# timmeinhardt/trackformer

Hardware: AMD Instinct MI355X
Metric: frames/sec, TrackFormer-Deformable inference (ResNet-50, 1333x800, 300 object + 100 track queries, bs 1 per GPU); roofline = ms_deform_attn HBM GB/s (higher is better)
Workload: dtype f32 (dense layers as the fp16 split product on MFMA: two fp16 pieces per activation, three per weight scaled per output channel -- 22 + 1 significand bits per operand, the one dropped product < 2^-22 --, three terms, f32 accumulate)

## Files before the change

include/tf_fused.h:

```cpp
#ifndef TF_FUSED_H_
#define TF_FUSED_H_

#include <stdint.h>

#ifdef __cplusplus
extern "C" {
#endif

int tf_bias_act_f32(float *x, const float *bias, const float *residual, int64_t n, int C, int relu,
                    void *stream);

int tf_add_layernorm_f32(const float *x, const float *res, const float *gamma, const float *beta,
                         float *out, int64_t rows, int C, float eps, void *stream);

int tf_box_refine_f32(const float *delta, const float *ref, float *out, int64_t rows, int ref_dim, float eps, void *stream);

int tf_postprocess_pack_f32(const float *logits, const float *boxes, float *out, int64_t Q, int C, float img_h, float img_w,
                            int clip, void *stream);

int tf_groupnorm_nhwc_f32(const float *x, const float *gamma, const float *beta, float *out, double *workspace, int N,
                          int HW, int C, int G, float eps, int64_t x_image_stride, int64_t out_image_stride, void *stream);
int tf_groupnorm_stats_nhwc_f32(const float *x, double *workspace, int N, int HW, int C, int G, int64_t x_image_stride, void *stream);
int tf_groupnorm_relu_nhwc_f32(const float *x, const float *gamma, const float *beta, float *out, double *workspace, int N,
                               int HW, int C, int G, float eps, int64_t x_image_stride, int64_t out_image_stride, void *stream);

int tf_upsample_add_nhwc_f32(const float *low, const float *fpn, float *out, int N, int q_per_image, int h, int w, int H, int W, int C,
                             void *stream);

int tf_conv3x3_merge_packed_f32(const float *low, const float *fpn, const double *gn_workspace, const float *gamma, const float *beta,
                                int groups, float eps, const void *w_packed, const float *bias, float *y, int nimg, int q_per_image, int lh,
                                int lw, int H, int W, int cin, int cout, int relu, int terms, void *stream);

int tf_groupnorm_relu_conv3x3_c1_nhwc_f32(const float *x, const float *gamma, const float *beta, const float *weight, float bias,
                                          float *out, double *workspace, int N, int H, int W, int C, int G, float eps, void *stream);

int tf_mask_label_map_f32(const float *logits, const int *order, int16_t *label, int n_tracks, int h, int w, int pad_h, int pad_w, int img_h,
                          int img_w, int out_h, int out_w, float threshold, void *stream);


int tf_linear_split_f32(const float *x, const void *w_hi, const void *w_mid, const void *w_lo, const float *w_scale, const float *bias,
                        float *y, int64_t M, int K, int N, int relu, void *stream);

int tf_linear_split_res_f32(const float *x, const void *w_hi, const void *w_mid, const void *w_lo, const float *w_scale, const float *bias,
                            const float *residual, float *y, int64_t M, int K, int N, int relu, void *stream);

int tf_conv3x3_split_f32(const float *x, const void *w_hi, const void *w_mid, const void *w_lo, const float *w_scale, const float *bias,
                         float *y, int nimg, int hin, int win, int cin, int cout, int stride, int relu, void *stream);
int tf_conv3x3_splitk_f32(const float *x, const void *w_hi, const void *w_mid, const void *w_lo, const float *w_scale, const float *bias,
                          float *y, float *workspace, int ksplit, int nimg, int hin, int win, int cin, int cout, int stride, int relu,
                          void *stream);
int tf_conv1x1_strided_split_f32(const float *x, const void *w_hi, const void *w_mid, const void *w_lo, const float *w_scale,
                                 const float *bias, float *y, int nimg, int hin, int win, int cin, int cout, int stride, int relu,
                                 void *stream);
int tf_conv1x1_splitk_f32(const float *x, const void *w_hi, const void *w_mid, const void *w_lo, const float *w_scale, const float *bias,
                          float *y, float *workspace, int ksplit, int nimg, int hin, int win, int cin, int cout, int stride, int relu,
                          void *stream);

int tf_stem_conv7x7_f32(const float *x, const void *w_packed, const float *bias, float *y, int N, int H, int W, int relu,
                        int terms, void *stream);

int tf_bias_relu_maxpool_f32(const float *x, const float *bias, float *out, int N, int H, int W, int C, void *stream);

int tf_linear_split_add_f32(const float *x, const float *x2, const void *w_hi, const void *w_mid, const void *w_lo, const float *w_scale,
                            const float *bias, float *y, int64_t M, int K, int N, void *stream);

int64_t tf_linear_packed_bytes(int K, int N, int terms);
int tf_linear_pack_weight_f32(const float *w, void *packed, int K, int N, int terms, void *stream);
int tf_linear_packed_f32(const float *x, const void *w_packed, const float *bias, const float *residual, float *y, int64_t M, int K,
                         int N, int relu, int terms, void *stream);

int tf_conv_packed_f32(const float *x, const void *w_packed, const float *bias, const float *residual, float *y, float *workspace,
                       int ksplit, int nimg, int hin, int win, int cin, int cout, int ks, int stride, int relu, int terms,
                       void *stream);

int tf_linear_res_ln_f32(const float *x, const void *w_packed, const float *bias, const float *residual, const float *ln_weight,
                         const float *ln_bias, float ln_eps, float *y, int64_t M, int K, int N, int terms, void *stream);

int tf_ffn_fused_f32(const float *x, const void *w1_packed, const float *b1, const void *w2_packed, const float *b2,
                     const float *residual, const float *ln_weight, const float *ln_bias, float ln_eps, float *y, int64_t M,
                     int d_model, int d_ffn, int terms, void *stream);

int tf_mha_core_f32(const float *q, const float *k, const float *v, float *out, const unsigned char *key_mask,
                    int N, int Lq, int Lk, int H, int D, int ldq, int ldk, int ldv, int ldo, float scale,
                    void *stream);

int tf_nms_host_f32(const float *boxes, const float *scores, int n, float iou_threshold, int64_t *keep, int *n_keep);

#ifdef __cplusplus
}
#endif
#endif
```

trackformer_amd/_cabi.py:

```python
import ctypes
import os

_PKG_DIR = os.path.dirname(os.path.abspath(__file__))
LIB_PATH = os.environ.get("TF_MSDA_LIB") or os.path.join(_PKG_DIR, "lib", "libtf_msda.so")

EXPORTED_SYMBOLS = (
    "tf_msda_abi_version",
    "tf_msda_strerror",
    "tf_msda_last_hip_error",
    "tf_msda_last_kernel",
    "tf_msda_set_tiled",
    "tf_msda_set_option",
    "tf_msda_debug_trace_buffer",
    "tf_msda_forward_fused_f32",
    "tf_msda_forward_f32",
    "tf_msda_forward_f64",
    "tf_msda_forward_f32_dshapes",
    "tf_msda_forward_f64_dshapes",
    "tf_msda_backward_f32",
    "tf_msda_backward_f64",
    "tf_msda_backward_f32_dshapes",
    "tf_msda_backward_f64_dshapes",
    "tf_msda_forward_host_f32",
    "tf_msda_forward_host_f64",
    "tf_msda_backward_host_f32",
    "tf_msda_backward_host_f64",
    "tf_bias_act_f32",
    "tf_add_layernorm_f32",
    "tf_groupnorm_nhwc_f32",
    "tf_groupnorm_relu_nhwc_f32",
    "tf_box_refine_f32",
    "tf_postprocess_pack_f32",
    "tf_upsample_add_nhwc_f32",
    "tf_mask_label_map_f32",
    "tf_conv3x3_merge_packed_f32",
    "tf_groupnorm_stats_nhwc_f32",
    "tf_groupnorm_relu_conv3x3_c1_nhwc_f32",
    "tf_bias_relu_maxpool_f32",
    "tf_stem_conv7x7_f32",
    "tf_linear_split_f32",
    "tf_linear_split_res_f32",
    "tf_conv3x3_split_f32",
    "tf_conv3x3_splitk_f32",
    "tf_conv1x1_strided_split_f32",
    "tf_conv1x1_splitk_f32",
    "tf_linear_packed_bytes",
    "tf_linear_pack_weight_f32",
    "tf_linear_packed_f32",
    "tf_linear_split_add_f32",
    "tf_ffn_fused_f32",
    "tf_linear_res_ln_f32",
    "tf_conv_packed_f32",
    "tf_mha_core_f32",
    "tf_nms_host_f32",
)

ABI_VERSION = 3

_lib = None


class MSDAError(RuntimeError):
    """Raised when libtf_msda.so reports a non-zero status."""


def lib():
    global _lib
    if _lib is not None:
        return _lib
    if not os.path.exists(LIB_PATH):
        raise RuntimeError(
            "trackformer_amd: native library %s not found. Build it with "
            "`python -m trackformer_amd.build` (needs hipcc); there is no CPU fallback." % LIB_PATH)
    import torch
    L = ctypes.CDLL(LIB_PATH)
    vp, ci = ctypes.c_void_p, ctypes.c_int
    L.tf_msda_abi_version.restype = ci
    L.tf_msda_abi_version.argtypes = []
    L.tf_msda_strerror.restype = ctypes.c_char_p
    L.tf_msda_strerror.argtypes = [ci]
    L.tf_msda_last_hip_error.restype = ci
    L.tf_msda_last_hip_error.argtypes = []
    L.tf_msda_last_kernel.restype = ctypes.c_char_p
    L.tf_msda_last_kernel.argtypes = []
    L.tf_msda_set_tiled.restype = ci
    L.tf_msda_set_tiled.argtypes = [ci]
    L.tf_msda_set_option.restype = ci
    L.tf_msda_set_option.argtypes = [ctypes.c_char_p, ci]
    L.tf_msda_debug_trace_buffer.restype = None
    L.tf_msda_debug_trace_buffer.argtypes = [vp]
    for suf in ("f32", "f64"):
        for tail in ("", "_dshapes"):
            f = getattr(L, "tf_msda_forward_%s%s" % (suf, tail))
            f.restype = ci
            f.argtypes = [vp] * 5 + [ci] * 7 + [vp]
            b = getattr(L, "tf_msda_backward_%s%s" % (suf, tail))
            b.restype = ci
            b.argtypes = [vp] * 8 + [ci] * 7 + [vp]
    for suf in ("f32", "f64"):
        f = getattr(L, "tf_msda_forward_host_" + suf)
        f.restype = ci
        f.argtypes = [vp] * 5 + [ci] * 7
        b = getattr(L, "tf_msda_backward_host_" + suf)
        b.restype = ci
        b.argtypes = [vp] * 8 + [ci] * 7
    L.tf_nms_host_f32.restype = ci
    L.tf_nms_host_f32.argtypes = [vp, vp, ci, ctypes.c_float, vp, vp]
    L.tf_msda_forward_fused_f32.restype = ci
    L.tf_msda_forward_fused_f32.argtypes = [vp, vp, vp, ci, vp, ci, ci, ci, vp] + [ci] * 7 + [vp]
    L.tf_bias_act_f32.restype = ci
    L.tf_bias_act_f32.argtypes = [vp, vp, vp, ctypes.c_int64, ci, ci, vp]
    L.tf_add_layernorm_f32.restype = ci
    L.tf_add_layernorm_f32.argtypes = [vp, vp, vp, vp, vp, ctypes.c_int64, ci, ctypes.c_float, vp]
    L.tf_stem_conv7x7_f32.restype = ci
    L.tf_stem_conv7x7_f32.argtypes = [vp, vp, vp, vp, ci, ci, ci, ci, ci, vp]
    L.tf_bias_relu_maxpool_f32.restype = ci
    L.tf_bias_relu_maxpool_f32.argtypes = [vp, vp, vp, ci, ci, ci, ci, vp]
    L.tf_box_refine_f32.restype = ci
    L.tf_box_refine_f32.argtypes = [vp, vp, vp, ctypes.c_int64, ci, ctypes.c_float, vp]
    L.tf_postprocess_pack_f32.restype = ci
    L.tf_postprocess_pack_f32.argtypes = [vp, vp, vp, ctypes.c_int64, ci, ctypes.c_float, ctypes.c_float, ci, vp]
    L.tf_groupnorm_stats_nhwc_f32.restype = ci
    L.tf_groupnorm_stats_nhwc_f32.argtypes = [vp, vp, ci, ci, ci, ci, ctypes.c_int64, vp]
    L.tf_conv3x3_merge_packed_f32.restype = ci
    L.tf_conv3x3_merge_packed_f32.argtypes = [vp, vp, vp, vp, vp, ci, ctypes.c_float, vp, vp, vp, ci, ci, ci, ci, ci, ci, ci, ci, ci, ci, vp]
    L.tf_mask_label_map_f32.restype = ci
    L.tf_mask_label_map_f32.argtypes = [vp, vp, vp, ci, ci, ci, ci, ci, ci, ci, ci, ci, ctypes.c_float, vp]
    L.tf_upsample_add_nhwc_f32.restype = ci
    L.tf_upsample_add_nhwc_f32.argtypes = [vp, vp, vp, ci, ci, ci, ci, ci, ci, ci, vp]
    L.tf_groupnorm_relu_conv3x3_c1_nhwc_f32.restype = ci
    L.tf_groupnorm_relu_conv3x3_c1_nhwc_f32.argtypes = [vp, vp, vp, vp, ctypes.c_float, vp, vp, ci, ci, ci, ci, ci, ctypes.c_float, vp]
    for fn in (L.tf_groupnorm_nhwc_f32, L.tf_groupnorm_relu_nhwc_f32):
        fn.restype = ci
        fn.argtypes = [vp, vp, vp, vp, vp, ci, ci, ci, ci, ctypes.c_float, ctypes.c_int64, ctypes.c_int64, vp]
    L.tf_linear_split_f32.restype = ci
    L.tf_linear_split_f32.argtypes = [vp, vp, vp, vp, vp, vp, vp, ctypes.c_int64, ci, ci, ci, vp]
    L.tf_linear_split_res_f32.restype = ci
    L.tf_linear_split_res_f32.argtypes = [vp, vp, vp, vp, vp, vp, vp, vp, ctypes.c_int64, ci, ci, ci, vp]
    L.tf_conv3x3_splitk_f32.restype = ci
    L.tf_conv3x3_splitk_f32.argtypes = [vp, vp, vp, vp, vp, vp, vp, vp, ci, ci, ci, ci, ci, ci, ci, ci, vp]
    L.tf_conv3x3_split_f32.restype = ci
    L.tf_conv3x3_split_f32.argtypes = [vp, vp, vp, vp, vp, vp, vp] + [ci] * 7 + [vp]
    L.tf_conv1x1_splitk_f32.restype = ci
    L.tf_conv1x1_splitk_f32.argtypes = [vp, vp, vp, vp, vp, vp, vp, vp, ci, ci, ci, ci, ci, ci, ci, ci, vp]
    L.tf_conv1x1_strided_split_f32.restype = ci
    L.tf_conv1x1_strided_split_f32.argtypes = [vp, vp, vp, vp, vp, vp, vp] + [ci] * 7 + [vp]
    L.tf_linear_packed_bytes.restype = ctypes.c_int64
    L.tf_linear_packed_bytes.argtypes = [ci, ci, ci]
    L.tf_linear_pack_weight_f32.restype = ci
    L.tf_linear_pack_weight_f32.argtypes = [vp, vp, ci, ci, ci, vp]
    L.tf_linear_res_ln_f32.restype = ci
    L.tf_linear_res_ln_f32.argtypes = [vp, vp, vp, vp, vp, vp, ctypes.c_float, vp, ctypes.c_int64, ci, ci, ci, vp]
    L.tf_ffn_fused_f32.restype = ci
    L.tf_ffn_fused_f32.argtypes = [vp, vp, vp, vp, vp, vp, vp, vp, ctypes.c_float, vp, ctypes.c_int64, ci, ci, ci, vp]
    L.tf_linear_split_add_f32.restype = ci
    L.tf_linear_split_add_f32.argtypes = [vp, vp, vp, vp, vp, vp, vp, vp, ctypes.c_int64, ci, ci, vp]
    L.tf_linear_packed_f32.restype = ci
    L.tf_linear_packed_f32.argtypes = [vp, vp, vp, vp, vp, ctypes.c_int64, ci, ci, ci, ci, vp]
    L.tf_conv_packed_f32.restype = ci
    L.tf_conv_packed_f32.argtypes = [vp, vp, vp, vp, vp, vp] + [ci] * 10 + [vp]
    L.tf_mha_core_f32.restype = ci
    L.tf_mha_core_f32.argtypes = [vp, vp, vp, vp, vp] + [ci] * 9 + [ctypes.c_float, vp]
    if L.tf_msda_abi_version() != ABI_VERSION:
        raise RuntimeError("libtf_msda.so ABI version %d != expected %d (rebuild)" %
                           (L.tf_msda_abi_version(), ABI_VERSION))
    _lib = L
    return _lib


def check(status, what):
    if status != 0:
        L = lib()
        msg = L.tf_msda_strerror(status).decode()
        raise MSDAError("%s failed: %s (status %d, hipError %d)" %
                        (what, msg, status, L.tf_msda_last_hip_error()))
```

trackformer_amd/build.py:

```python
import hashlib
import os
import shutil
import subprocess
import sys
from concurrent.futures import ThreadPoolExecutor

PKG_DIR = os.path.dirname(os.path.abspath(__file__))
REPO_DIR = os.path.dirname(PKG_DIR)
CSRC = os.path.join(PKG_DIR, "csrc")
LIB_DIR = os.path.join(PKG_DIR, "lib")
INCLUDE = os.path.join(REPO_DIR, "include")
GFX_ARCH = "gfx950"

_TARGETS = [
    ("libtf_msda.so", ["msda_hip.hip", "msda_pquad.hip", "fused_ops.hip", "linear_split.hip", "linear_stream.hip", "mha_core.hip", "ffn_fused.hip", "stem_conv.hip", "msda_host.cpp"], []),
]


def _hipcc():
    exe = shutil.which("hipcc") or "/opt/rocm/bin/hipcc"
    if not os.path.exists(exe):
        raise RuntimeError("hipcc not found (expected on PATH or at /opt/rocm/bin/hipcc)")
    return exe


def _key(deps, flags):
    h = hashlib.sha256()
    h.update(("\0".join(flags) + "\0" + GFX_ARCH).encode())
    for d in sorted(deps):
        h.update(os.path.basename(d).encode())
        with open(d, "rb") as f:
            h.update(f.read())
    return h.hexdigest()


def _stale(out, key):
    stamp = out + ".stamp"
    if not os.path.exists(out) or not os.path.exists(stamp):
        return True
    with open(stamp) as f:
        return f.read().strip() != key


def _stamp(out, key):
    with open(out + ".stamp", "w") as f:
        f.write(key + "\n")


def _run(cmd, verbose):
    if verbose:
        print(" ".join(cmd), flush=True)
    subprocess.check_call(cmd)


def build_all(force=False, verbose=False):
    os.makedirs(LIB_DIR, exist_ok=True)
    built = []
    headers = [os.path.join(INCLUDE, f) for f in os.listdir(INCLUDE) if f.endswith(".h")]
    headers += [os.path.join(CSRC, f) for f in os.listdir(CSRC) if f.endswith(".h")]
    for out_name, srcs, extra in _TARGETS:
        out = os.path.join(LIB_DIR, out_name)
        src_paths = [os.path.join(CSRC, s) for s in srcs]
        flags = ["--offload-arch=" + GFX_ARCH, "-O3", "-std=c++17", "-fPIC", "-I" + INCLUDE,
                 "-Wno-pass-failed"] + extra
        key = _key(src_paths + headers, flags)
        if not force and not _stale(out, key):
            continue
        obj_dir = os.path.join(LIB_DIR, "obj")
        os.makedirs(obj_dir, exist_ok=True)
        objs = [os.path.join(obj_dir, os.path.splitext(s)[0] + ".o") for s in srcs]
        with ThreadPoolExecutor(max_workers=len(srcs)) as pool:
            list(pool.map(lambda so: _run([_hipcc()] + flags + ["-c", so[0], "-o", so[1]], verbose),
                          zip(src_paths, objs)))
        _run([_hipcc(), "--offload-arch=" + GFX_ARCH, "-shared", "-fPIC", "-pthread"] + objs + ["-o", out], verbose)
        _stamp(out, key)
        built.append(out)
    built += _build_tools(force, verbose)
    return built


def _build_tools(force, verbose):
    out_dir = os.path.join(REPO_DIR, "tools", "bin")
    lib = os.path.join(LIB_DIR, "libtf_msda.so")
    built = []
    for name in ("msda_bench", "linear_bench", "ffn_bench"):
        src = os.path.join(REPO_DIR, "tools", name + ".cpp")
        if not os.path.exists(src):
            continue
        os.makedirs(out_dir, exist_ok=True)
        out = os.path.join(out_dir, name)
        flags = ["--offload-arch=" + GFX_ARCH, "-O2", "-std=c++17", "-I" + INCLUDE]
        headers = [os.path.join(INCLUDE, f) for f in os.listdir(INCLUDE) if f.endswith(".h")]
        key = _key([src] + headers, flags)
        if not force and not _stale(out, key) and os.path.getmtime(out) >= os.path.getmtime(lib):
            continue
        _run([_hipcc()] + flags + [src, "-L" + LIB_DIR, "-ltf_msda",
                                   "-Wl,-rpath,$ORIGIN/../../trackformer_amd/lib", "-o", out], verbose)
        _stamp(out, key)
        built.append(out)
    return built


if __name__ == "__main__":
    res = build_all(force="--force" in sys.argv, verbose=True)
    print("built:" if res else "up to date", *res)
```

trackformer_amd/csrc/ffn_fused.hip:

```cpp
#include <hip/hip_runtime.h>

#include <stdint.h>
#include <stdlib.h>

#include <atomic>
#include <type_traits>

#include "msda_common.h"
#include "split_product.h"
#include "tf_fused.h"
#include "tf_msda.h"

namespace {

template <int D>
struct Geo {
    static_assert(D == 256 || D == 288, "hidden sizes of the reference's configurations");
    static constexpr int NW = D == 256 ? 4 : 3;
    static constexpr int NT = NW * 64;
    static constexpr int TJ = D / 32 / NW;
    static constexpr int XS = D + 8;
    static constexpr int CH = NW * 32;
    static constexpr int HS = CH + 8;
    static constexpr int KQ1 = D / 16;
    static constexpr int U1 = KQ1 / 2;
    static constexpr int U2 = CH / 16;
    static constexpr int UPC = U1 + U2;
    static constexpr int us(int nb) { return nb * (TJ > 2 ? TJ : 2); }
    static constexpr int RING = D == 256 ? 8 : 5;
    static constexpr int AHEAD = RING - 2;
    static_assert(TJ * NW * 32 == D && KQ1 % 2 == 0 && UPC % RING == 0, "geometry");
};

template <int... I, class F>
__device__ __forceinline__ void static_for_impl(std::integer_sequence<int, I...>, F &&f)
{
    (f(std::integral_constant<int, I>{}), ...);
}
template <int N, class F>
__device__ __forceinline__ void static_for(F &&f)
{
    static_for_impl(std::make_integer_sequence<int, N>{}, f);
}

template <int D>
constexpr size_t ffn_lds_bytes(int ti, int na) { return (size_t)(32 * ti) * (Geo<D>::XS + Geo<D>::HS) * 2 * na; }

template <int SP, int D, int TI>
__device__ __forceinline__ void stage_rows(const float *__restrict__ X, int M, int m0, unsigned short *sX, int tid)
{
    using G = Geo<D>;
    constexpr int C4 = D / 4, NV = TI * 32 * C4 / G::NT;
    static_assert(TI * 32 * C4 % G::NT == 0, "tile does not divide among the threads");
    f32x4 xr[NV];
#pragma unroll
    for (int it = 0; it < NV; ++it) {
        const int idx = it * G::NT + tid;
        const int row = idx / C4, c4 = idx - row * C4;
        const int grow = min(m0 + row, M - 1);
        xr[it] = *reinterpret_cast<const f32x4 *>(X + (size_t)grow * D + c4 * 4);
    }
    __builtin_amdgcn_sched_barrier(0);
#pragma unroll
    for (int it = 0; it < NV; ++it) {
        const int idx = it * G::NT + tid;
        const int row = idx / C4, c4 = idx - row * C4;
        u32x2 pc[Split<SP>::NA];
        split4<SP>(xr[it], pc);
#pragma unroll
        for (int p = 0; p < Split<SP>::NA; ++p) *reinterpret_cast<u32x2 *>(&sX[(p * TI * 32 + row) * G::XS + c4 * 4]) = pc[p];
    }
}

template <int NW>
__device__ __forceinline__ float wave_partials(const float *s, int stride)
{
    if constexpr (NW == 4) return (s[0] + s[stride]) + (s[2 * stride] + s[3 * stride]);
    else return (s[0] + s[stride]) + s[2 * stride];
}

template <int D, int TI, bool LN, bool F16>
__device__ __forceinline__ void rows_epilogue(const f32x16 (&accy)[TI][Geo<D>::TJ], f32x4 (&v)[TI][Geo<D>::TJ][4],
                                              const __amdgpu_buffer_rsrc_t b2rs, const float *__restrict__ r, const float *__restrict__ gamma,
                                              const float *__restrict__ beta, float eps, const __amdgpu_buffer_rsrc_t yrs, float *sRed,
                                              int m0, int wave, int lane)
{
    using G = Geo<D>;
    constexpr int BM = TI * 32, TJ = G::TJ, NW = G::NW;
    const int frow = lane & 31, cbase = wave * (32 * TJ) + 4 * (lane >> 5);
#pragma unroll
    for (int j = 0; j < TJ; ++j)
#pragma unroll
        for (int g = 0; g < 4; ++g) {
            const f32x4 b = __builtin_bit_cast(f32x4, __builtin_amdgcn_raw_buffer_load_b128(b2rs, (unsigned)(cbase + 32 * j + 8 * g) * 4u, 0, 0));
            f32x4 rv = {1.f, 1.f, 1.f, 1.f};
            if constexpr (F16) rv = *reinterpret_cast<const f32x4 *>(r + cbase + 32 * j + 8 * g);
#pragma unroll
            for (int i = 0; i < TI; ++i)
#pragma unroll
                for (int e = 0; e < 4; ++e)
                    v[i][j][g][e] = (F16 ? __builtin_fmaf(accy[i][j][4 * g + e], rv[e], b[e]) : accy[i][j][4 * g + e] + b[e]) + v[i][j][g][e];
        }
    if constexpr (LN) {
        float s[TI];
#pragma unroll
        for (int i = 0; i < TI; ++i) {
            float a = 0.f;
#pragma unroll
            for (int j = 0; j < TJ; ++j)
#pragma unroll
                for (int g = 0; g < 4; ++g) a += (v[i][j][g].x + v[i][j][g].y) + (v[i][j][g].z + v[i][j][g].w);
            s[i] = a + __shfl_xor(a, 32);
        }
        __syncthreads();
        if (lane < 32)
#pragma unroll
            for (int i = 0; i < TI; ++i) sRed[wave * BM + i * 32 + lane] = s[i];
        __syncthreads();
        float mean[TI], rstd[TI];
#pragma unroll
        for (int i = 0; i < TI; ++i) {
            mean[i] = wave_partials<NW>(sRed + i * 32 + frow, BM) * (1.f / D);
            float a = 0.f;
#pragma unroll
            for (int j = 0; j < TJ; ++j)
#pragma unroll
                for (int g = 0; g < 4; ++g) {
                    const f32x4 d = v[i][j][g] - mean[i];
                    a += (d.x * d.x + d.y * d.y) + (d.z * d.z + d.w * d.w);
                }
            s[i] = a + __shfl_xor(a, 32);
        }
        if (lane < 32)
#pragma unroll
            for (int i = 0; i < TI; ++i) sRed[(NW + wave) * BM + i * 32 + lane] = s[i];
        __syncthreads();
#pragma unroll
        for (int i = 0; i < TI; ++i) rstd[i] = rsqrtf(wave_partials<NW>(sRed + NW * BM + i * 32 + frow, BM) * (1.f / D) + eps);
#pragma unroll
        for (int j = 0; j < TJ; ++j)
#pragma unroll
            for (int g = 0; g < 4; ++g) {
                const f32x4 ga = *reinterpret_cast<const f32x4 *>(gamma + cbase + 32 * j + 8 * g);
                const f32x4 be = *reinterpret_cast<const f32x4 *>(beta + cbase + 32 * j + 8 * g);
#pragma unroll
                for (int i = 0; i < TI; ++i) v[i][j][g] = (v[i][j][g] - mean[i]) * rstd[i] * ga + be;
            }
    }
#pragma unroll
    for (int i = 0; i < TI; ++i)
#pragma unroll
        for (int j = 0; j < TJ; ++j)
#pragma unroll
            for (int g = 0; g < 4; ++g)
                __builtin_amdgcn_raw_buffer_store_b128(__builtin_bit_cast(u32x4, v[i][j][g]), yrs,
                                                       (unsigned)((m0 + i * 32 + frow) * D + cbase + 32 * j + 8 * g) * 4u, 0, tfm::kStoreAux);
}

template <int SP, int D, int TI, bool LN>
__global__ void __launch_bounds__(Geo<D>::NT, 1)
ffn_fused_kernel(const float *__restrict__ X, const u32x4 *__restrict__ W1p, const float *__restrict__ b1,
                 const u32x4 *__restrict__ W2p, const float *__restrict__ b2, const float *R,
                 const float *__restrict__ gamma, const float *__restrict__ beta, float eps, float *Y, int M, int F)
{
    using G = Geo<D>;
    constexpr int BM = TI * 32, TJ = G::TJ, NW = G::NW, XS = G::XS, HS = G::HS, RING = G::RING, UPC = G::UPC, U1 = G::U1, U2 = G::U2;
    constexpr int NA = Split<SP>::NA, NB = Split<SP>::NB, US = G::us(NB);
    constexpr bool F16 = Split<SP>::F16;
    extern __shared__ __attribute__((aligned(16))) unsigned short s_f[];
    unsigned short *const sX = s_f;
    unsigned short *const sH = s_f + NA * BM * XS;
    const int tid = threadIdx.x, lane = tid & 63;
    const int wave = __builtin_amdgcn_readfirstlane(tid >> 6);
    const int m0 = blockIdx.x * BM;
    const int nchunks = (F + G::CH - 1) / G::CH, KQ2 = F >> 4;
    const int ntiles1 = (F + 255) / 256 * 8;

    u32x4 ring[RING][US];
    auto load_unit = [&](int c, auto uc, u32x4 (&dst)[US]) {
        constexpr int u = decltype(uc)::value;
        if constexpr (u < U1) {
            const u32x4 *base = W1p + ((size_t)min(c * NW + wave, ntiles1 - 1) * G::KQ1 * NB + u * 2 * NB) * 64 + lane;
#pragma unroll
            for (int i = 0; i < 2 * NB; ++i) dst[i] = base[i * 64];
        } else {
            const int q = min(c * U2 + (u - U1), KQ2 - 1);
#pragma unroll
            for (int j = 0; j < TJ; ++j)
#pragma unroll
                for (int p = 0; p < NB; ++p) dst[j * NB + p] = W2p[(((size_t)(TJ * wave + j) * KQ2 + q) * NB + p) * 64 + lane];
        }
    };
    static_for<G::AHEAD>([&](auto uc) { load_unit(0, uc, ring[decltype(uc)::value]); });
    __builtin_amdgcn_sched_barrier(0);
    stage_rows<SP, D, TI>(X, M, m0, sX, tid);
    __syncthreads();

    f32x16 accy[TI][TJ];
#pragma unroll
    for (int i = 0; i < TI; ++i)
#pragma unroll
        for (int j = 0; j < TJ; ++j)
#pragma unroll
            for (int e = 0; e < 16; ++e) accy[i][j][e] = 0.f;

    const float *const r1 = reinterpret_cast<const float *>(W1p + (size_t)ntiles1 * G::KQ1 * NB * 64);
    const float *const r2 = reinterpret_cast<const float *>(W2p + (size_t)((D + 255) / 256 * 8) * KQ2 * NB * 64);
    const int frow = (lane & 31), fk = (lane >> 5) * 8;
    const int xoff = frow * XS + fk, hoff = frow * HS + fk;

    const __amdgpu_buffer_rsrc_t b1rs = __builtin_amdgcn_make_buffer_rsrc(const_cast<float *>(b1 ? b1 : X), 0, b1 ? (unsigned)F * 4u : 0u, 0x00020000);
    const __amdgpu_buffer_rsrc_t b2rs = __builtin_amdgcn_make_buffer_rsrc(const_cast<float *>(b2 ? b2 : X), 0, b2 ? (unsigned)D * 4u : 0u, 0x00020000);
    const unsigned bytes = (unsigned)((size_t)M * D * 4);
    const __amdgpu_buffer_rsrc_t yrs = __builtin_amdgcn_make_buffer_rsrc(Y, 0, bytes, 0x00020000);
    const __amdgpu_buffer_rsrc_t rrs = __builtin_amdgcn_make_buffer_rsrc(const_cast<float *>(R ? R : X), 0, R ? bytes : 0u, 0x00020000);
    const int cbase = wave * (32 * TJ) + 4 * (lane >> 5);
    f32x4 v[TI][TJ][4];

    for (int c = 0; c < nchunks; ++c) {
        const int cn = min(c + 1, nchunks - 1);
        f32x4 b1v[4], r1v[4];
#pragma unroll
        for (int g = 0; g < 4; ++g) {
            r1v[g] = f32x4{1.f, 1.f, 1.f, 1.f};
            b1v[g] = __builtin_bit_cast(f32x4, __builtin_amdgcn_raw_buffer_load_b128(
                                                   b1rs, (unsigned)(c * G::CH + wave * 32 + 8 * g + 4 * (lane >> 5)) * 4u, 0, 0));
            if constexpr (F16)
                r1v[g] = *reinterpret_cast<const f32x4 *>(r1 + min(c * G::CH + wave * 32 + 8 * g + 4 * (lane >> 5), ntiles1 * 32 - 4));
        }
        if (c == nchunks - 1) {
#pragma unroll
            for (int i = 0; i < TI; ++i)
#pragma unroll
                for (int j = 0; j < TJ; ++j)
#pragma unroll
                    for (int g = 0; g < 4; ++g)
                        v[i][j][g] = __builtin_bit_cast(f32x4, __builtin_amdgcn_raw_buffer_load_b128(
                                                                   rrs, (unsigned)((m0 + i * 32 + frow) * D + cbase + 32 * j + 8 * g) * 4u, 0, 0));
        }
        f32x16 acch[TI][1];
#pragma unroll
        for (int i = 0; i < TI; ++i)
#pragma unroll
            for (int e = 0; e < 16; ++e) acch[i][0][e] = 0.f;

        auto prefetch = [&](auto uc) {
            constexpr int ahead = decltype(uc)::value + G::AHEAD;
            if constexpr (ahead < UPC) load_unit(c, std::integral_constant<int, ahead>{}, ring[ahead % RING]);
            else load_unit(cn, std::integral_constant<int, ahead - UPC>{}, ring[ahead % RING]);
        };
        u32x4 xf[2][TI][NA];
        auto read_x = [&](auto stc) {
            constexpr int st = decltype(stc)::value;
#pragma unroll
            for (int i = 0; i < TI; ++i)
#pragma unroll
                for (int p = 0; p < NA; ++p)
                    xf[st & 1][i][p] = *reinterpret_cast<const u32x4 *>(&sX[(p * BM + i * 32) * XS + xoff + st * 16]);
        };
        read_x(std::integral_constant<int, 0>{});
        static_for<G::KQ1>([&](auto stc) {
            constexpr int st = decltype(stc)::value;
            if constexpr ((st & 1) == 0) prefetch(std::integral_constant<int, st / 2>{});
            if constexpr (st + 1 < G::KQ1) read_x(std::integral_constant<int, st + 1>{});
            __builtin_amdgcn_sched_barrier(0);
            const u32x4 (&cur)[US] = ring[(st / 2) % RING];
            u32x4 wf[1][NB];
#pragma unroll
            for (int p = 0; p < NB; ++p) wf[0][p] = cur[(st & 1) * NB + p];
            mfma_tiles<SP, TI, 1, false>(acch, xf[st & 1], wf);
        });

        __syncthreads();
        const int hcol = c * G::CH + wave * 32 + 4 * (lane >> 5);
#pragma unroll
        for (int i = 0; i < TI; ++i)
#pragma unroll
            for (int g = 0; g < 4; ++g) {
                f32x4 hv;
#pragma unroll
                for (int e = 0; e < 4; ++e) {
                    const float t = F16 ? __builtin_fmaf(acch[i][0][4 * g + e], r1v[g][e], b1v[g][e]) : acch[i][0][4 * g + e] + b1v[g][e];
                    hv[e] = (t < 0.f || hcol + 8 * g >= F) ? 0.f : t;
                }
                u32x2 pc[NA];
                split4<SP>(hv, pc);
                const int o = (i * 32 + frow) * HS + wave * 32 + 8 * g + 4 * (lane >> 5);
#pragma unroll
                for (int p = 0; p < NA; ++p) *reinterpret_cast<u32x2 *>(&sH[p * BM * HS + o]) = pc[p];
            }
        __syncthreads();

        u32x4 hf[2][TI][NA];
        auto read_h = [&](auto vc) {
            constexpr int kv = decltype(vc)::value;
#pragma unroll
            for (int i = 0; i < TI; ++i)
#pragma unroll
                for (int p = 0; p < NA; ++p)
                    hf[kv & 1][i][p] = *reinterpret_cast<const u32x4 *>(&sH[(p * BM + i * 32) * HS + hoff + kv * 16]);
        };
        read_h(std::integral_constant<int, 0>{});
        static_for<U2>([&](auto vc) {
            constexpr int kv = decltype(vc)::value;
            prefetch(std::integral_constant<int, U1 + kv>{});
            if constexpr (kv + 1 < U2) read_h(std::integral_constant<int, kv + 1>{});
            __builtin_amdgcn_sched_barrier(0);
            const u32x4 (&cur)[US] = ring[(U1 + kv) % RING];
            u32x4 wf[TJ][NB];
#pragma unroll
            for (int j = 0; j < TJ; ++j)
#pragma unroll
                for (int p = 0; p < NB; ++p) wf[j][p] = cur[j * NB + p];
            mfma_tiles<SP, TI, TJ, false>(accy, hf[kv & 1], wf);
        });
    }

    rows_epilogue<D, TI, LN, F16>(accy, v, b2rs, r2, gamma, beta, eps, yrs, reinterpret_cast<float *>(sH), m0, wave, lane);
}

template <int SP, int D, int TI>
int launch_ffn(const float *x, const u32x4 *w1, const float *b1, const u32x4 *w2, const float *b2, const float *res,
               const float *gamma, const float *beta, float eps, float *y, int M, int F, hipStream_t s)
{
    const bool ln = gamma != nullptr;
    constexpr size_t lds = ffn_lds_bytes<D>(TI, Split<SP>::NA);
    static_assert(lds <= 160 * 1024, "the two tiles do not fit the LDS of a CU");
    const void *fn = ln ? (const void *)&ffn_fused_kernel<SP, D, TI, true> : (const void *)&ffn_fused_kernel<SP, D, TI, false>;
    static std::atomic<unsigned> raised[2];
    int dev = 0;
    (void)hipGetDevice(&dev);
    if (dev >= 32 || !(raised[ln ? 1 : 0].load() & (1u << dev))) {
        if (hipFuncSetAttribute(fn, hipFuncAttributeMaxDynamicSharedMemorySize, (int)lds) != hipSuccess) return TF_MSDA_ERR_LAUNCH;
        if (dev < 32) raised[ln ? 1 : 0].fetch_or(1u << dev);
    }
    const int blocks = (M + 32 * TI - 1) / (32 * TI);
    void *argv[] = {(void *)&x, (void *)&w1, (void *)&b1, (void *)&w2, (void *)&b2, (void *)&res,
                    (void *)&gamma, (void *)&beta, (void *)&eps, (void *)&y, (void *)&M, (void *)&F};
    return hipLaunchKernel(fn, dim3((unsigned)blocks), dim3(Geo<D>::NT), argv, lds, s) == hipSuccess ? TF_MSDA_OK : TF_MSDA_ERR_LAUNCH;
}

template <int D>
constexpr size_t linln_lds_bytes(int ti, int na) { return (size_t)(32 * ti) * Geo<D>::XS * 2 * na; }
constexpr int linln_min_blocks(int d, int ti) { return (d == 256 ? ti <= 2 : ti <= 1) ? 2 : 1; }
constexpr int linln_ring(int ti) { return ti <= 2 ? 4 : 8; }

template <int SP, int D, int TI, bool LN>
__global__ void __launch_bounds__(Geo<D>::NT, (linln_min_blocks(D, TI)))
linear_res_ln_kernel(const float *__restrict__ X, const u32x4 *__restrict__ Wp, const float *__restrict__ bias, const float *R,
                     const float *__restrict__ gamma, const float *__restrict__ beta, float eps, float *Y, int M)
{
    using G = Geo<D>;
    constexpr int BM = TI * 32, TJ = G::TJ, XS = G::XS, KQ = G::KQ1, NA = Split<SP>::NA, NB = Split<SP>::NB;
    extern __shared__ __attribute__((aligned(16))) unsigned short s_f[];
    unsigned short *const sX = s_f;
    const int tid = threadIdx.x, lane = tid & 63;
    const int wave = __builtin_amdgcn_readfirstlane(tid >> 6);
    const int m0 = blockIdx.x * BM;
    constexpr int RING = linln_ring(TI), AHEAD = RING - 2;
    u32x4 ring[RING][NB * TJ];
    auto load_unit = [&](auto uc, u32x4 (&dst)[NB * TJ]) {
        constexpr int u = decltype(uc)::value;
#pragma unroll
        for (int j = 0; j < TJ; ++j)
#pragma unroll
            for (int p = 0; p < NB; ++p) dst[j * NB + p] = Wp[(((size_t)(TJ * wave + j) * KQ + u) * NB + p) * 64 + lane];
    };
    static_for<AHEAD>([&](auto uc) { load_unit(uc, ring[decltype(uc)::value]); });
    __builtin_amdgcn_sched_barrier(0);
    const __amdgpu_buffer_rsrc_t brs = __builtin_amdgcn_make_buffer_rsrc(const_cast<float *>(bias ? bias : X), 0, bias ? (unsigned)D * 4u : 0u, 0x00020000);
    const unsigned bytes = (unsigned)((size_t)M * D * 4);
    const __amdgpu_buffer_rsrc_t yrs = __builtin_amdgcn_make_buffer_rsrc(Y, 0, bytes, 0x00020000);
    const __amdgpu_buffer_rsrc_t rrs = __builtin_amdgcn_make_buffer_rsrc(const_cast<float *>(R ? R : X), 0, R ? bytes : 0u, 0x00020000);
    const int frow = lane & 31, cbase = wave * (32 * TJ) + 4 * (lane >> 5);
    f32x4 v[TI][TJ][4];
    stage_rows<SP, D, TI>(X, M, m0, sX, tid);
    __syncthreads();

    f32x16 accy[TI][TJ];
#pragma unroll
    for (int i = 0; i < TI; ++i)
#pragma unroll
        for (int j = 0; j < TJ; ++j)
#pragma unroll
            for (int e = 0; e < 16; ++e) accy[i][j][e] = 0.f;
    const int xoff = frow * XS + (lane >> 5) * 8;
    u32x4 xf[2][TI][NA];
    auto read_x = [&](auto stc) {
        constexpr int st = decltype(stc)::value;
#pragma unroll
        for (int i = 0; i < TI; ++i)
#pragma unroll
            for (int p = 0; p < NA; ++p)
                xf[st & 1][i][p] = *reinterpret_cast<const u32x4 *>(&sX[(p * BM + i * 32) * XS + xoff + st * 16]);
    };
    read_x(std::integral_constant<int, 0>{});
    static_for<KQ>([&](auto stc) {
        constexpr int st = decltype(stc)::value;
        if constexpr (st + AHEAD < KQ) load_unit(std::integral_constant<int, st + AHEAD>{}, ring[(st + AHEAD) % RING]);
        if constexpr (st == KQ - AHEAD) {
#pragma unroll
            for (int i = 0; i < TI; ++i)
#pragma unroll
                for (int j = 0; j < TJ; ++j)
#pragma unroll
                    for (int g = 0; g < 4; ++g)
                        v[i][j][g] = __builtin_bit_cast(f32x4, __builtin_amdgcn_raw_buffer_load_b128(
                                                                   rrs, (unsigned)((m0 + i * 32 + frow) * D + cbase + 32 * j + 8 * g) * 4u, 0, 0));
        }
        if constexpr (st + 1 < KQ) read_x(std::integral_constant<int, st + 1>{});
        __builtin_amdgcn_sched_barrier(0);
        const u32x4 (&cur)[NB * TJ] = ring[st % RING];
        u32x4 wf[TJ][NB];
#pragma unroll
        for (int j = 0; j < TJ; ++j)
#pragma unroll
            for (int p = 0; p < NB; ++p) wf[j][p] = cur[j * NB + p];
        mfma_tiles<SP, TI, TJ, false>(accy, xf[st & 1], wf);
    });
    const float *const r = reinterpret_cast<const float *>(Wp + (size_t)((D + 255) / 256 * 8) * KQ * NB * 64);
    rows_epilogue<D, TI, LN, Split<SP>::F16>(accy, v, brs, r, gamma, beta, eps, yrs, reinterpret_cast<float *>(sX), m0, wave, lane);
}

template <int SP, int D, int TI>
int launch_linln(const float *x, const u32x4 *w, const float *b, const float *res, const float *gamma, const float *beta, float eps,
                 float *y, int M, hipStream_t s)
{
    const bool ln = gamma != nullptr;
    constexpr size_t lds = linln_lds_bytes<D>(TI, Split<SP>::NA);
    static_assert(lds <= 160 * 1024, "the activation tile does not fit the LDS of a CU");
    const void *fn = ln ? (const void *)&linear_res_ln_kernel<SP, D, TI, true> : (const void *)&linear_res_ln_kernel<SP, D, TI, false>;
    if (lds > 64 * 1024) {
        static std::atomic<unsigned> raised[2];
        int dev = 0;
        (void)hipGetDevice(&dev);
        if (dev >= 32 || !(raised[ln ? 1 : 0].load() & (1u << dev))) {
            if (hipFuncSetAttribute(fn, hipFuncAttributeMaxDynamicSharedMemorySize, (int)lds) != hipSuccess) return TF_MSDA_ERR_LAUNCH;
            if (dev < 32) raised[ln ? 1 : 0].fetch_or(1u << dev);
        }
    }
    const int blocks = (M + 32 * TI - 1) / (32 * TI);
    void *argv[] = {(void *)&x, (void *)&w, (void *)&b, (void *)&res, (void *)&gamma, (void *)&beta, (void *)&eps, (void *)&y, (void *)&M};
    return hipLaunchKernel(fn, dim3((unsigned)blocks), dim3(Geo<D>::NT), argv, lds, s) == hipSuccess ? TF_MSDA_OK : TF_MSDA_ERR_LAUNCH;
}

std::atomic<int> g_linln_ti{-1};
int linln_ti()
{
    int v = g_linln_ti.load(std::memory_order_relaxed);
    if (v < 0) {
        const char *e = getenv("TF_LINLN_TI");
        v = e ? atoi(e) : 0;
        if (v < 0 || v > 3) v = 0;
        g_linln_ti.store(v);
    }
    return v;
}

std::atomic<int> g_ffn_tail{-1};
std::atomic<int> g_ffn_ti{-1};
int ffn_ti()
{
    int v = g_ffn_ti.load(std::memory_order_relaxed);
    if (v < 0) {
        const char *e = getenv("TF_FFN_TI");
        v = e ? atoi(e) : 3;
        if (v < 1 || v > 3) v = 3;
        g_ffn_ti.store(v);
    }
    return v;
}

}

namespace tfm {
int ffn_tail_split()
{
    int v = g_ffn_tail.load(std::memory_order_relaxed);
    if (v < 0) {
        const char *e = getenv("TF_FFN_TAIL_SPLIT");
        v = (e && e[0] == '0') ? 0 : 1;
        g_ffn_tail.store(v);
    }
    return v;
}
int ffn_set_tail_split(int v)
{
    const int prev = ffn_tail_split();
    g_ffn_tail.store(v ? 1 : 0);
    return prev;
}
int ffn_set_ti(int v)
{
    const int prev = ffn_ti();
    g_ffn_ti.store(v >= 1 && v <= 3 ? v : 3);
    return prev;
}
int linln_set_ti(int v)
{
    const int prev = linln_ti();
    g_linln_ti.store(v >= 1 && v <= 3 ? v : 0);
    return prev;
}
}

namespace {

int ffn_num_cus()
{
    static const int n = [] {
        int dev = 0, cus = 256;
        if (hipGetDevice(&dev) == hipSuccess) {
            hipDeviceProp_t prop;
            if (hipGetDeviceProperties(&prop, dev) == hipSuccess && prop.multiProcessorCount > 0) cus = prop.multiProcessorCount;
        }
        return cus;
    }();
    return n;
}

template <int SP, int D>
int dispatch_linln(const float *x, const u32x4 *w, const float *bias, const float *residual, const float *g, const float *b, float eps,
                   float *y, int M, hipStream_t s)
{
    const int forced = linln_ti();
    switch (forced ? forced : (M < 4096 || Split<SP>::NA == 3 ? 1 : (SP == 16 && D == 256 ? 3 : 2))) {
    case 1: return launch_linln<SP, D, 1>(x, w, bias, residual, g, b, eps, y, M, s);
    case 3:
        if constexpr (D == 256 && Split<SP>::NB == 2) return launch_linln<SP, D, 3>(x, w, bias, residual, g, b, eps, y, M, s);
        else return launch_linln<SP, D, 2>(x, w, bias, residual, g, b, eps, y, M, s);
    default: return launch_linln<SP, D, 2>(x, w, bias, residual, g, b, eps, y, M, s);
    }
}

template <int SP, int D>
int dispatch_ffn(const float *x, const u32x4 *w1, const float *b1, const u32x4 *w2, const float *b2, const float *residual,
                 const float *g, const float *b, float eps, float *y, int M, int F, hipStream_t s)
{
    if (F < Geo<D>::CH || (F & 15)) return TF_MSDA_ERR_BAD_DIMS;
    constexpr bool three_tiles = D == 256 && Split<SP>::NB == 2;
    const int want = ffn_ti();
    const bool ti2 = want == 2 || (want >= 3 && !three_tiles);
    if (ti2 && tfm::ffn_tail_split()) {
        const int cus = ffn_num_cus();
        const long long per_round = 64LL * cus;
        const int main_rows = (int)(M / per_round * per_round), rem = M - main_rows;
        if (main_rows > 0 && rem > 0 && rem <= 32LL * cus) {
            int rc = launch_ffn<SP, D, 2>(x, w1, b1, w2, b2, residual, g, b, eps, y, main_rows, F, s);
            if (rc != TF_MSDA_OK) return rc;
            const size_t off = (size_t)main_rows * D;
            return launch_ffn<SP, D, 1>(x + off, w1, b1, w2, b2, residual ? residual + off : nullptr, g, b, eps, y + off, rem, F, s);
        }
    }
    switch (want) {
    case 1: return launch_ffn<SP, D, 1>(x, w1, b1, w2, b2, residual, g, b, eps, y, M, F, s);
    case 2: return launch_ffn<SP, D, 2>(x, w1, b1, w2, b2, residual, g, b, eps, y, M, F, s);
    default:
        if constexpr (three_tiles) return launch_ffn<SP, D, 3>(x, w1, b1, w2, b2, residual, g, b, eps, y, M, F, s);
        else return launch_ffn<SP, D, 2>(x, w1, b1, w2, b2, residual, g, b, eps, y, M, F, s);
    }
}

template <int D>
int dispatch_linln_scheme(int sp, const float *x, const u32x4 *w, const float *bias, const float *residual, const float *g, const float *b,
                          float eps, float *y, int M, hipStream_t s)
{
    switch (sp) {
    case 3: return dispatch_linln<3, D>(x, w, bias, residual, g, b, eps, y, M, s);
    default: return dispatch_linln<16, D>(x, w, bias, residual, g, b, eps, y, M, s);
    }
}

template <int D>
int dispatch_ffn_scheme(int sp, const float *x, const u32x4 *w1, const float *b1, const u32x4 *w2, const float *b2, const float *residual,
                        const float *g, const float *b, float eps, float *y, int M, int F, hipStream_t s)
{
    switch (sp) {
    case 3: return dispatch_ffn<3, D>(x, w1, b1, w2, b2, residual, g, b, eps, y, M, F, s);
    default: return dispatch_ffn<16, D>(x, w1, b1, w2, b2, residual, g, b, eps, y, M, F, s);
    }
}

}

extern "C" int tf_linear_res_ln_f32(const float *x, const void *w_packed, const float *bias, const float *residual,
                                    const float *ln_weight, const float *ln_bias, float ln_eps, float *y, int64_t M, int K, int N,
                                    int terms, void *stream)
{
    if (!x || !w_packed || !y) return TF_MSDA_ERR_NULL_POINTER;
    if ((ln_weight == nullptr) != (ln_bias == nullptr)) return TF_MSDA_ERR_NULL_POINTER;
    const int sp = split_scheme(terms);
    if (M <= 0 || K != N || (K != 256 && K != 288) || (M + 128) * (int64_t)K * 4 > 0xFFFFFFFFLL || sp == 0) return TF_MSDA_ERR_BAD_DIMS;
    uintptr_t al = reinterpret_cast<uintptr_t>(x) | reinterpret_cast<uintptr_t>(w_packed) | reinterpret_cast<uintptr_t>(y) |
                   reinterpret_cast<uintptr_t>(bias) | reinterpret_cast<uintptr_t>(residual) | reinterpret_cast<uintptr_t>(ln_weight) |
                   reinterpret_cast<uintptr_t>(ln_bias);
    if (al & 15) return TF_MSDA_ERR_BAD_DIMS;
    const u32x4 *w = static_cast<const u32x4 *>(w_packed);
    hipStream_t s = static_cast<hipStream_t>(stream);
    return K == 256 ? dispatch_linln_scheme<256>(sp, x, w, bias, residual, ln_weight, ln_bias, ln_eps, y, (int)M, s)
                    : dispatch_linln_scheme<288>(sp, x, w, bias, residual, ln_weight, ln_bias, ln_eps, y, (int)M, s);
}

extern "C" int tf_ffn_fused_f32(const float *x, const void *w1_packed, const float *b1, const void *w2_packed, const float *b2,
                                const float *residual, const float *ln_weight, const float *ln_bias, float ln_eps, float *y,
                                int64_t M, int d_model, int d_ffn, int terms, void *stream)
{
    if (!x || !w1_packed || !w2_packed || !y) return TF_MSDA_ERR_NULL_POINTER;
    if ((ln_weight == nullptr) != (ln_bias == nullptr)) return TF_MSDA_ERR_NULL_POINTER;
    const int sp = split_scheme(terms);
    if (M <= 0 || (d_model != 256 && d_model != 288) || d_ffn <= 0 || sp == 0 ||
        (M + 128) * (int64_t)d_model * 4 > 0xFFFFFFFFLL)
        return TF_MSDA_ERR_BAD_DIMS;
    uintptr_t al = reinterpret_cast<uintptr_t>(x) | reinterpret_cast<uintptr_t>(w1_packed) | reinterpret_cast<uintptr_t>(w2_packed) |
                   reinterpret_cast<uintptr_t>(y) | reinterpret_cast<uintptr_t>(b1) | reinterpret_cast<uintptr_t>(b2) |
                   reinterpret_cast<uintptr_t>(residual) | reinterpret_cast<uintptr_t>(ln_weight) | reinterpret_cast<uintptr_t>(ln_bias);
    if (al & 15) return TF_MSDA_ERR_BAD_DIMS;
    const u32x4 *w1 = static_cast<const u32x4 *>(w1_packed), *w2 = static_cast<const u32x4 *>(w2_packed);
    hipStream_t s = static_cast<hipStream_t>(stream);
    return d_model == 256 ? dispatch_ffn_scheme<256>(sp, x, w1, b1, w2, b2, residual, ln_weight, ln_bias, ln_eps, y, (int)M, d_ffn, s)
                          : dispatch_ffn_scheme<288>(sp, x, w1, b1, w2, b2, residual, ln_weight, ln_bias, ln_eps, y, (int)M, d_ffn, s);
}
```

trackformer_amd/csrc/linear_split.hip:

```cpp
#include <hip/hip_runtime.h>

#include <stdint.h>
#include <stdlib.h>

#include <atomic>
#include <type_traits>

#include "msda_common.h"
#include "split_product.h"
#include "tf_fused.h"
#include "tf_msda.h"

namespace {

constexpr int BK = 32, THREADS = 256;
constexpr int LDS_STRIDE = BK + 8;

__device__ __forceinline__ int stage_row(int q) { return (q & ~7) | ((q & 1) << 2) | ((q & 7) >> 1); }

template <int SP, int BM, int BN, bool RELU, bool PREFETCH, bool RESID, bool BUFST, bool XADD = false>
__device__ __forceinline__ void
split_gemm_body(const float *__restrict__ X, const unsigned short *__restrict__ Whi,
                const unsigned short *__restrict__ Wmid, const unsigned short *__restrict__ Wlo, const float *__restrict__ Wsc,
                const float *__restrict__ bias, const float *__restrict__ R, float *__restrict__ Y, int M, int K, int N,
                const float *__restrict__ X2 = nullptr)
{
    constexpr int NA = Split<SP>::NA, NB = Split<SP>::NB;
    constexpr bool F16 = Split<SP>::F16;
    const unsigned short *const Wp[3] = {Whi, Wmid, Wlo};
    constexpr int TI = BM / 64, TJ = BN / 64;
    constexpr int XV = (BM * BK / 4) / THREADS;
    constexpr int WV = (BN * BK / 8) / THREADS;
    static_assert(XV >= 1 && WV >= 1, "tile too small for 256 threads");
    __shared__ __attribute__((aligned(16))) unsigned short sA[NA][BM * LDS_STRIDE];
    __shared__ __attribute__((aligned(16))) unsigned short sB[NB][BN * LDS_STRIDE];
    const int tid = threadIdx.x, lane = tid & 63, wave = tid >> 6;
    const int m0 = blockIdx.x * BM, n0 = blockIdx.y * BN;
    const int wm = (wave >> 1) * (BM / 2), wn = (wave & 1) * (BN / 2);

    f32x16 acc[TI][TJ];
#pragma unroll
    for (int i = 0; i < TI; ++i)
#pragma unroll
        for (int j = 0; j < TJ; ++j)
#pragma unroll
            for (int r = 0; r < 16; ++r) acc[i][j][r] = 0.f;

    f32x4 xr[XV];
    u32x4 wr[NB][WV];
    f32x4 xr2[XADD ? XV : 1];
    auto load_slice = [&](int k0) {
#pragma unroll
        for (int it = 0; it < XV; ++it) {
            const int idx = it * THREADS + tid;
            const int row = stage_row(idx >> 3), c4 = idx & 7;
            const int grow = min(m0 + row, M - 1);
            xr[it] = *reinterpret_cast<const f32x4 *>(X + (size_t)grow * K + k0 + c4 * 4);
            if constexpr (XADD) xr2[it] = *reinterpret_cast<const f32x4 *>(X2 + (size_t)grow * K + k0 + c4 * 4);
        }
#pragma unroll
        for (int it = 0; it < WV; ++it) {
            const int idx = it * THREADS + tid;
            const int row = stage_row(idx >> 2), c8 = idx & 3;
            const int grow = min(n0 + row, N - 1);
            const size_t g = (size_t)grow * K + k0 + c8 * 8;
#pragma unroll
            for (int q = 0; q < NB; ++q) wr[q][it] = *reinterpret_cast<const u32x4 *>(Wp[q] + g);
        }
    };
    auto store_slice = [&]() {
#pragma unroll
        for (int it = 0; it < XV; ++it) {
            const int idx = it * THREADS + tid;
            const int row = stage_row(idx >> 3), c4 = idx & 7;
            u32x2 pc[NA];
            f32x4 xv = xr[it];
            if constexpr (XADD) xv += xr2[it];
            split4<SP>(xv, pc);
#pragma unroll
            for (int q = 0; q < NA; ++q) *reinterpret_cast<u32x2 *>(&sA[q][row * LDS_STRIDE + c4 * 4]) = pc[q];
        }
#pragma unroll
        for (int it = 0; it < WV; ++it) {
            const int idx = it * THREADS + tid;
            const int row = stage_row(idx >> 2), c8 = idx & 3;
#pragma unroll
            for (int q = 0; q < NB; ++q) *reinterpret_cast<u32x4 *>(&sB[q][row * LDS_STRIDE + c8 * 8]) = wr[q][it];
        }
    };

    if constexpr (PREFETCH) load_slice(0);
    for (int k0 = 0; k0 < K; k0 += BK) {
        if constexpr (!PREFETCH) load_slice(k0);
        store_slice();
        __syncthreads();
        if constexpr (PREFETCH)
            if (k0 + BK < K) load_slice(k0 + BK);
#pragma unroll
        for (int kk = 0; kk < BK; kk += 16) {
            const int koff = kk + (lane >> 5) * 8;
            u32x4 af[TI][NA], bfr[TJ][NB];
#pragma unroll
            for (int i = 0; i < TI; ++i) {
                const int r = (wm + i * 32 + (lane & 31)) * LDS_STRIDE + koff;
#pragma unroll
                for (int q = 0; q < NA; ++q) af[i][q] = *reinterpret_cast<const u32x4 *>(&sA[q][r]);
            }
#pragma unroll
            for (int j = 0; j < TJ; ++j) {
                const int r = (wn + j * 32 + (lane & 31)) * LDS_STRIDE + koff;
#pragma unroll
                for (int q = 0; q < NB; ++q) bfr[j][q] = *reinterpret_cast<const u32x4 *>(&sB[q][r]);
            }
            mfma_tiles<SP, TI, TJ>(acc, af, bfr);
        }
        __syncthreads();
    }
    if constexpr (BUFST) {
        const unsigned ybytes = (unsigned)((size_t)M * N * 4);
        const __amdgpu_buffer_rsrc_t yrs = __builtin_amdgcn_make_buffer_rsrc(Y, 0, ybytes, 0x00020000);
        const __amdgpu_buffer_rsrc_t rrs = __builtin_amdgcn_make_buffer_rsrc(const_cast<float *>(RESID ? R : Y), 0, ybytes, 0x00020000);
#pragma unroll
        for (int i = 0; i < TI; ++i)
#pragma unroll
            for (int j = 0; j < TJ; ++j) {
                const int col = n0 + wn + j * 32 + (lane & 31);
                const bool colok = col < N;
                const float b = (bias && colok) ? bias[col] : 0.f;
                const float rsc = (F16 && colok) ? Wsc[col] : 1.f;
                const int row0 = m0 + wm + i * 32 + 4 * (lane >> 5);
                const unsigned base = colok ? (unsigned)(row0 * N + col) * 4u : 0xC0000000u;
                float rv[16];
                if constexpr (RESID) {
#pragma unroll
                    for (int r = 0; r < 16; ++r) {
                        const unsigned off = base + (unsigned)(((r & 3) + 8 * (r >> 2)) * N) * 4u;
                        rv[r] = __builtin_bit_cast(float, __builtin_amdgcn_raw_buffer_load_b32(rrs, off, 0, 0));
                    }
                }
#pragma unroll
                for (int r = 0; r < 16; ++r) {
                    float v = F16 ? __builtin_fmaf(acc[i][j][r], rsc, b) : acc[i][j][r] + b;
                    if constexpr (RESID) v += rv[r];
                    if (RELU) v = v < 0.f ? 0.f : v;
                    const unsigned off = base + (unsigned)(((r & 3) + 8 * (r >> 2)) * N) * 4u;
                    __builtin_amdgcn_raw_buffer_store_b32(__builtin_bit_cast(unsigned, v), yrs, off, 0, tfm::kStoreAux);
                }
            }
        return;
    }
#pragma unroll
    for (int i = 0; i < TI; ++i)
#pragma unroll
        for (int j = 0; j < TJ; ++j) {
            const int col = n0 + wn + j * 32 + (lane & 31);
            if (col >= N) continue;
            const float b = bias ? bias[col] : 0.f;
            const float rsc = F16 ? Wsc[col] : 1.f;
#pragma unroll
            for (int r = 0; r < 16; ++r) {
                const int row = m0 + wm + i * 32 + (r & 3) + 8 * (r >> 2) + 4 * (lane >> 5);
                if (row < M) {
                    float v = F16 ? __builtin_fmaf(acc[i][j][r], rsc, b) : acc[i][j][r] + b;
                    if constexpr (RESID) v += R[(size_t)row * N + col];
                    if (RELU) v = v < 0.f ? 0.f : v;
                    Y[(size_t)row * N + col] = v;
                }
            }
        }
}

template <int SP, int BM, int BN, bool RELU, bool PREFETCH, bool BUFST = false>
__global__ void __launch_bounds__(THREADS)
split_gemm_kernel(const float *__restrict__ X, const unsigned short *__restrict__ Whi,
                  const unsigned short *__restrict__ Wmid, const unsigned short *__restrict__ Wlo, const float *__restrict__ Wsc,
                  const float *__restrict__ bias, float *__restrict__ Y, int M, int K, int N)
{
    split_gemm_body<SP, BM, BN, RELU, PREFETCH, false, BUFST>(X, Whi, Wmid, Wlo, Wsc, bias, nullptr, Y, M, K, N);
}

template <int SP, int BM, int BN, bool RELU, bool PREFETCH, bool BUFST = false>
__global__ void __launch_bounds__(THREADS)
split_gemm_res_kernel(const float *__restrict__ X, const unsigned short *__restrict__ Whi,
                      const unsigned short *__restrict__ Wmid, const unsigned short *__restrict__ Wlo, const float *__restrict__ Wsc,
                      const float *__restrict__ bias, const float *__restrict__ R, float *__restrict__ Y, int M, int K, int N)
{
    split_gemm_body<SP, BM, BN, RELU, PREFETCH, true, BUFST>(X, Whi, Wmid, Wlo, Wsc, bias, R, Y, M, K, N);
}

template <int SP, int BM, int BN, bool PREFETCH, bool BUFST>
__global__ void __launch_bounds__(THREADS)
split_gemm_add_kernel(const float *__restrict__ X, const float *__restrict__ X2, const unsigned short *__restrict__ Whi,
                      const unsigned short *__restrict__ Wmid, const unsigned short *__restrict__ Wlo, const float *__restrict__ Wsc,
                      const float *__restrict__ bias, float *__restrict__ Y, int M, int K, int N)
{
    split_gemm_body<SP, BM, BN, false, PREFETCH, false, BUFST, true>(X, Whi, Wmid, Wlo, Wsc, bias, nullptr, Y, M, K, N, X2);
}

struct Conv3Args {
    int nimg, hin, win, cin, hout, wout, cout, stride;
    int ks, pad;
    int kslices;
};

template <int SP, int BM, int BN, bool RELU>
__global__ void __launch_bounds__(THREADS)
split_conv3_kernel(const float *__restrict__ X, const unsigned short *__restrict__ Whi,
                   const unsigned short *__restrict__ Wmid, const unsigned short *__restrict__ Wlo, const float *__restrict__ Wsc,
                   const float *__restrict__ bias, float *__restrict__ Y, const Conv3Args ca)
{
    constexpr int NA = Split<SP>::NA, NB = Split<SP>::NB;
    constexpr bool F16 = Split<SP>::F16;
    constexpr int TI = BM / 64, TJ = BN / 64;
    constexpr int XV = (BM * BK / 4) / THREADS;
    constexpr int WV = (BN * BK / 8) / THREADS;
    static_assert(XV >= 1 && WV >= 1, "tile too small for 256 threads");
    __shared__ __attribute__((aligned(16))) unsigned short sA[NA][BM * LDS_STRIDE];
    __shared__ __attribute__((aligned(16))) unsigned short sB[NB][BN * LDS_STRIDE];
    const int tid = threadIdx.x, lane = tid & 63, wave = tid >> 6;
    const int m0 = blockIdx.x * BM, n0 = blockIdx.y * BN;
    const int wm = (wave >> 1) * (BM / 2), wn = (wave & 1) * (BN / 2);
    const int M = ca.nimg * ca.hout * ca.wout, K = ca.ks * ca.ks * ca.cin, N = ca.cout;

    f32x16 acc[TI][TJ];
#pragma unroll
    for (int i = 0; i < TI; ++i)
#pragma unroll
        for (int j = 0; j < TJ; ++j)
#pragma unroll
            for (int r = 0; r < 16; ++r) acc[i][j][r] = 0.f;

    int ybase[XV], xbase[XV];
    bool rowok[XV];
    f32x4 xr[XV];
    u32x4 wr[NB][WV];
    constexpr unsigned OOB = 0xC0000000u;
    unsigned xoff[XV], woff[WV];
    const __amdgpu_buffer_rsrc_t xrs = __builtin_amdgcn_make_buffer_rsrc(
        const_cast<float *>(X), 0, (unsigned)((size_t)ca.nimg * ca.hin * ca.win * ca.cin * 4), 0x00020000);
    const unsigned wbytes = (unsigned)((size_t)N * K * 2);
    const __amdgpu_buffer_rsrc_t wrs[3] = {
        __builtin_amdgcn_make_buffer_rsrc(const_cast<unsigned short *>(Whi), 0, wbytes, 0x00020000),
        __builtin_amdgcn_make_buffer_rsrc(const_cast<unsigned short *>(Wmid), 0, wbytes, 0x00020000),
        __builtin_amdgcn_make_buffer_rsrc(const_cast<unsigned short *>(NB > 2 ? Wlo : Whi), 0, wbytes, 0x00020000)};
#pragma unroll
    for (int it = 0; it < XV; ++it) {
        const int idx = it * THREADS + tid;
        const int row = m0 + (stage_row(idx >> 3));
        rowok[it] = row < M;
        const int r = rowok[it] ? row : 0;
        const int img = r / (ca.hout * ca.wout), rem = r - img * (ca.hout * ca.wout);
        const int yo = rem / ca.wout, xo = rem - yo * ca.wout;
        ybase[it] = yo * ca.stride - ca.pad;
        xbase[it] = xo * ca.stride - ca.pad;
        xoff[it] = ((unsigned)((img * ca.hin + ybase[it]) * ca.win + xbase[it]) * (unsigned)ca.cin + (unsigned)((idx & 7) * 4)) * 4u;
    }
#pragma unroll
    for (int it = 0; it < WV; ++it) {
        const int idx = it * THREADS + tid;
        woff[it] = ((unsigned)min(n0 + (stage_row(idx >> 2)), N - 1) * (unsigned)K + (unsigned)((idx & 3) * 8)) * 2u;
    }
    int nc0 = 0, ndx = 0, ndy = 0;
    auto load_slice = [&](int k0) {
        const int c0 = nc0, dx = ndx, dy = ndy;
        nc0 += BK;
        if (nc0 == ca.cin) {
            nc0 = 0;
            if (++ndx == ca.ks) {
                ndx = 0;
                ++ndy;
            }
        }
        const unsigned tapoff = (unsigned)((dy * ca.win + dx) * ca.cin + c0) * 4u;
#pragma unroll
        for (int it = 0; it < XV; ++it) {
            const bool ok = rowok[it] && (unsigned)(ybase[it] + dy) < (unsigned)ca.hin && (unsigned)(xbase[it] + dx) < (unsigned)ca.win;
            xr[it] = __builtin_bit_cast(f32x4, __builtin_amdgcn_raw_buffer_load_b128(xrs, ok ? xoff[it] + tapoff : OOB, 0, 0));
        }
#pragma unroll
        for (int it = 0; it < WV; ++it) {
            const unsigned o = woff[it] + (unsigned)k0 * 2u;
#pragma unroll
            for (int q = 0; q < NB; ++q) wr[q][it] = __builtin_amdgcn_raw_buffer_load_b128(wrs[q], o, 0, 0);
        }
    };
    auto store_slice = [&]() {
#pragma unroll
        for (int it = 0; it < XV; ++it) {
            const int idx = it * THREADS + tid;
            const int row = stage_row(idx >> 3), c4 = idx & 7;
            u32x2 pc[NA];
            split4<SP>(xr[it], pc);
#pragma unroll
            for (int q = 0; q < NA; ++q) *reinterpret_cast<u32x2 *>(&sA[q][row * LDS_STRIDE + c4 * 4]) = pc[q];
        }
#pragma unroll
        for (int it = 0; it < WV; ++it) {
            const int idx = it * THREADS + tid;
            const int row = stage_row(idx >> 2), c8 = idx & 3;
#pragma unroll
            for (int q = 0; q < NB; ++q) *reinterpret_cast<u32x4 *>(&sB[q][row * LDS_STRIDE + c8 * 8]) = wr[q][it];
        }
    };

    const int kbeg = ca.kslices > 0 ? (int)blockIdx.z * ca.kslices * BK : 0;
    const int kend = ca.kslices > 0 ? min(K, kbeg + ca.kslices * BK) : K;
    if (ca.kslices > 0) Y += (size_t)blockIdx.z * M * N;
    {
        const int tap = kbeg / ca.cin;
        nc0 = kbeg - tap * ca.cin;
        ndy = tap / ca.ks;
        ndx = tap - ndy * ca.ks;
    }
    load_slice(kbeg);
    for (int k0 = kbeg; k0 < kend; k0 += BK) {
        store_slice();
        __syncthreads();
        if (k0 + BK < kend) load_slice(k0 + BK);
#pragma unroll
        for (int kk = 0; kk < BK; kk += 16) {
            const int koff = kk + (lane >> 5) * 8;
            u32x4 af[TI][NA], bfr[TJ][NB];
#pragma unroll
            for (int i = 0; i < TI; ++i) {
                const int r = (wm + i * 32 + (lane & 31)) * LDS_STRIDE + koff;
#pragma unroll
                for (int q = 0; q < NA; ++q) af[i][q] = *reinterpret_cast<const u32x4 *>(&sA[q][r]);
            }
#pragma unroll
            for (int j = 0; j < TJ; ++j) {
                const int r = (wn + j * 32 + (lane & 31)) * LDS_STRIDE + koff;
#pragma unroll
                for (int q = 0; q < NB; ++q) bfr[j][q] = *reinterpret_cast<const u32x4 *>(&sB[q][r]);
            }
            mfma_tiles<SP, TI, TJ>(acc, af, bfr);
        }
        __syncthreads();
    }
    const __amdgpu_buffer_rsrc_t yrs = __builtin_amdgcn_make_buffer_rsrc(Y, 0, (unsigned)((size_t)M * N * 4), 0x00020000);
#pragma unroll
    for (int i = 0; i < TI; ++i)
#pragma unroll
        for (int j = 0; j < TJ; ++j) {
            const int col = n0 + wn + j * 32 + (lane & 31);
            const bool colok = col < N;
            const float b = (bias && colok) ? bias[col] : 0.f;
            const float rsc = (F16 && colok) ? Wsc[col] : 1.f;
            const int row0 = m0 + wm + i * 32 + 4 * (lane >> 5);
            const unsigned base = colok ? (unsigned)(row0 * N + col) * 4u : 0xC0000000u;
// ... 53 lines not shown

    f32x16 acc;
#pragma unroll
    for (int r = 0; r < 16; ++r) acc[r] = 0.f;

    f32x4 xr[PFD][XV];
    u32x4 wr[PFD][NB][WV];
    const float *xp[XV];
    size_t wg[WV];
#pragma unroll
    for (int it = 0; it < XV; ++it) {
        const int idx = it * THREADS + tid;
        const int row = stage_row(idx >> 3), c4 = idx & 7;
        xp[it] = X + (size_t)min(m0 + row, M - 1) * K + c4 * 4;
    }
#pragma unroll
    for (int it = 0; it < WV; ++it) {
        const int idx = it * THREADS + tid;
        const int row = stage_row(idx >> 2), c8 = idx & 3;
        wg[it] = (size_t)min(n0 + row, N - 1) * K + c8 * 8;
    }
    auto load_slice = [&](int s, auto slotc) {
        constexpr int slot = decltype(slotc)::value;
#pragma unroll
        for (int it = 0; it < XV; ++it) xr[slot][it] = *reinterpret_cast<const f32x4 *>(xp[it] + s * BK);
#pragma unroll
        for (int it = 0; it < WV; ++it)
#pragma unroll
            for (int q = 0; q < NB; ++q) wr[slot][q][it] = *reinterpret_cast<const u32x4 *>(Wp[q] + wg[it] + s * BK);
    };
    auto store_slice = [&](auto slotc, int buf) {
        constexpr int slot = decltype(slotc)::value;
#pragma unroll
        for (int it = 0; it < XV; ++it) {
            const int idx = it * THREADS + tid;
            const int row = stage_row(idx >> 3), c4 = idx & 7;
            u32x2 pc[NA];
            split4<SP>(xr[slot][it], pc);
#pragma unroll
            for (int q = 0; q < NA; ++q) *reinterpret_cast<u32x2 *>(&sA[buf][q][row * LDS_STRIDE + c4 * 4]) = pc[q];
        }
#pragma unroll
        for (int it = 0; it < WV; ++it) {
            const int idx = it * THREADS + tid;
            const int row = stage_row(idx >> 2), c8 = idx & 3;
#pragma unroll
            for (int q = 0; q < NB; ++q) *reinterpret_cast<u32x4 *>(&sB[buf][q][row * LDS_STRIDE + c8 * 8]) = wr[slot][q][it];
        }
    };
    auto each_slot = [&](auto &&f) {
        f(std::integral_constant<int, 0>{});
        f(std::integral_constant<int, 1>{});
        f(std::integral_constant<int, 2>{});
        f(std::integral_constant<int, 3>{});
        f(std::integral_constant<int, 4>{});
        f(std::integral_constant<int, 5>{});
        f(std::integral_constant<int, 6>{});
        f(std::integral_constant<int, 7>{});
    };

    static_assert(S >= PFD, "at least one full ring");
    each_slot([&](auto jc) { load_slice(decltype(jc)::value, jc); });
    store_slice(std::integral_constant<int, 0>{}, 0);
    __syncthreads();
    auto step = [&](auto sc) {
        constexpr int sidx = decltype(sc)::value;
        if constexpr (sidx < S) {
            constexpr int j = sidx % PFD, buf = sidx & 1;
            if constexpr (sidx + 1 < S) store_slice(std::integral_constant<int, (j + 1) % PFD>{}, buf ^ 1);
            if constexpr (sidx + PFD < S) load_slice(sidx + PFD, std::integral_constant<int, j>{});
#pragma unroll
            for (int kk = 0; kk < BK; kk += 16) {
                const int koff = kk + (lane >> 5) * 8;
                const int ra = (wm + (lane & 31)) * LDS_STRIDE + koff, rb = (wn + (lane & 31)) * LDS_STRIDE + koff;
                u32x4 af[NA], bfr[NB];
#pragma unroll
                for (int q = 0; q < NA; ++q) af[q] = *reinterpret_cast<const u32x4 *>(&sA[buf][q][ra]);
#pragma unroll
                for (int q = 0; q < NB; ++q) bfr[q] = *reinterpret_cast<const u32x4 *>(&sB[buf][q][rb]);
                mfma_terms<SP>(acc, af, bfr);
            }
            __syncthreads();
        }
    };
    auto steps4 = [&](auto bc) {
        constexpr int b = decltype(bc)::value;
        step(std::integral_constant<int, b>{});
        step(std::integral_constant<int, b + 1>{});
        step(std::integral_constant<int, b + 2>{});
        step(std::integral_constant<int, b + 3>{});
    };
    static_assert(S <= 36, "unrolled for up to 36 slices");
    steps4(std::integral_constant<int, 0>{});
    steps4(std::integral_constant<int, 4>{});
    steps4(std::integral_constant<int, 8>{});
    steps4(std::integral_constant<int, 12>{});
    steps4(std::integral_constant<int, 16>{});
    steps4(std::integral_constant<int, 20>{});
    steps4(std::integral_constant<int, 24>{});
    steps4(std::integral_constant<int, 28>{});
    steps4(std::integral_constant<int, 32>{});
    const __amdgpu_buffer_rsrc_t yrs = __builtin_amdgcn_make_buffer_rsrc(Y, 0, (unsigned)((size_t)M * N * 4), 0x00020000);
    const int col = n0 + wn + (lane & 31);
    const bool colok = col < N;
    const float b = (bias && colok) ? bias[col] : 0.f;
    const float rsc = (Split<SP>::F16 && colok) ? Wsc[col] : 1.f;
    const int row0 = m0 + wm + 4 * (lane >> 5);
    const unsigned base = colok ? (unsigned)(row0 * N + col) * 4u : 0xC0000000u;
#pragma unroll
    for (int r = 0; r < 16; ++r) {
        float v = Split<SP>::F16 ? __builtin_fmaf(acc[r], rsc, b) : acc[r] + b;
        if (RELU) v = v < 0.f ? 0.f : v;
        __builtin_amdgcn_raw_buffer_store_b32(__builtin_bit_cast(unsigned, v), yrs,
                                              base + (unsigned)(((r & 3) + 8 * (r >> 2)) * N) * 4u, 0, tfm::kStoreAux);
    }
}

inline bool fits_bufstore(long long M, int N) { return (M + 256) * N * 4 < 0xC0000000LL; }

struct Weight {
    const unsigned short *p[3];
    const float *scale;
};

template <int SP, int BM, int BN, bool PREFETCH>
int launch_gemm(const float *x, const Weight &w, const float *bias, const float *res, float *y, int M, int K, int N, int relu, hipStream_t s)
{
    const dim3 grid((unsigned)((M + BM - 1) / BM), (unsigned)((N + BN - 1) / BN));
    if (grid.y > 65535u) return TF_MSDA_ERR_BAD_DIMS;
    auto go = [&](auto bufst) {
        constexpr bool B = decltype(bufst)::value;
        if (res) {
            if (relu) hipLaunchKernelGGL((split_gemm_res_kernel<SP, BM, BN, true, PREFETCH, B>), grid, dim3(THREADS), 0, s, x, w.p[0], w.p[1], w.p[2], w.scale, bias, res, y, M, K, N);
            else hipLaunchKernelGGL((split_gemm_res_kernel<SP, BM, BN, false, PREFETCH, B>), grid, dim3(THREADS), 0, s, x, w.p[0], w.p[1], w.p[2], w.scale, bias, res, y, M, K, N);
        } else {
            if (relu) hipLaunchKernelGGL((split_gemm_kernel<SP, BM, BN, true, PREFETCH, B>), grid, dim3(THREADS), 0, s, x, w.p[0], w.p[1], w.p[2], w.scale, bias, y, M, K, N);
            else hipLaunchKernelGGL((split_gemm_kernel<SP, BM, BN, false, PREFETCH, B>), grid, dim3(THREADS), 0, s, x, w.p[0], w.p[1], w.p[2], w.scale, bias, y, M, K, N);
        }
    };
    if (fits_bufstore(M, N)) go(std::true_type{});
    else go(std::false_type{});
    return hipGetLastError() == hipSuccess ? TF_MSDA_OK : TF_MSDA_ERR_LAUNCH;
}

template <int SP, int BM, int BN, bool PREFETCH>
int launch_add(const float *x, const float *x2, const Weight &w, const float *bias, float *y, int M, int K, int N, hipStream_t s)
{
    const dim3 grid((unsigned)((M + BM - 1) / BM), (unsigned)((N + BN - 1) / BN));
    if (grid.y > 65535u) return TF_MSDA_ERR_BAD_DIMS;
    if (fits_bufstore(M, N))
        hipLaunchKernelGGL((split_gemm_add_kernel<SP, BM, BN, PREFETCH, true>), grid, dim3(THREADS), 0, s, x, x2, w.p[0], w.p[1], w.p[2], w.scale, bias, y, M, K, N);
    else
        hipLaunchKernelGGL((split_gemm_add_kernel<SP, BM, BN, PREFETCH, false>), grid, dim3(THREADS), 0, s, x, x2, w.p[0], w.p[1], w.p[2], w.scale, bias, y, M, K, N);
    return hipGetLastError() == hipSuccess ? TF_MSDA_OK : TF_MSDA_ERR_LAUNCH;
}

inline int weight_scheme(const void *w_hi, const void *w_mid, const void *w_lo, const float *w_scale, Weight &w)
{
    if (!w_hi || !w_mid) return 0;
    if (w_scale && w_lo) return -1;
    if ((reinterpret_cast<uintptr_t>(w_hi) | reinterpret_cast<uintptr_t>(w_mid) | reinterpret_cast<uintptr_t>(w_lo)) & 15) return -1;
    w.p[0] = static_cast<const unsigned short *>(w_hi);
    w.p[1] = static_cast<const unsigned short *>(w_mid);
    w.p[2] = static_cast<const unsigned short *>(w_lo);
    w.scale = w_scale;
    if (!w_scale && !w_lo) return -1;
    return w_scale ? 16 : 3;
}

template <class F>
int with_scheme(int sp, F &&f)
{
    switch (sp) {
    case 3: return f(std::integral_constant<int, 3>{});
    default: return f(std::integral_constant<int, 16>{});
    }
}

template <int SP>
int linear_split_sp(const float *x, const Weight &w, const float *bias, const float *res, float *y, int M, int K, int N, int relu,
                    hipStream_t s)
{
    if (M <= 4096) {
        if (!res && fits_bufstore(M, N)) {
            const dim3 grid((unsigned)((M + 63) / 64), (unsigned)((N + 63) / 64));
            if (grid.y > 65535u) return TF_MSDA_ERR_BAD_DIMS;
            const int slices = K / BK;
#define TF_DEEP(SS)                                                                                                                               \
    if (slices == SS) {                                                                                                                           \
        if (relu)                                                                                                                                 \
            hipLaunchKernelGGL((split_gemm_deep_kernel<SP, true, SS>), grid, dim3(THREADS), 0, s, x, w.p[0], w.p[1], w.p[2], w.scale, bias, y, M, K, N);  \
        else                                                                                                                                      \
            hipLaunchKernelGGL((split_gemm_deep_kernel<SP, false, SS>), grid, dim3(THREADS), 0, s, x, w.p[0], w.p[1], w.p[2], w.scale, bias, y, M, K, N); \
        return hipGetLastError() == hipSuccess ? TF_MSDA_OK : TF_MSDA_ERR_LAUNCH;                                                                 \
    }
            TF_DEEP(8) TF_DEEP(9) TF_DEEP(32) TF_DEEP(36)
#undef TF_DEEP
        }
        return launch_gemm<SP, 64, 64, true>(x, w, bias, res, y, M, K, N, relu, s);
    }
    if (K >= 512 && N <= 256) return launch_gemm<SP, 128, 64, true>(x, w, bias, res, y, M, K, N, relu, s);
    if (N > 256 && N < 512) return launch_gemm<SP, 64, 128, false>(x, w, bias, res, y, M, K, N, relu, s);
    return launch_gemm<SP, 64, 128, true>(x, w, bias, res, y, M, K, N, relu, s);
}

int linear_split_impl(const float *x, const void *w_hi, const void *w_mid, const void *w_lo, const float *w_scale, const float *bias,
                      const float *res, float *y, int64_t M, int K, int N, int relu, void *stream)
{
    if (!x || !y) return TF_MSDA_ERR_NULL_POINTER;
    Weight w;
    const int sp = weight_scheme(w_hi, w_mid, w_lo, w_scale, w);
    if (sp == 0) return TF_MSDA_ERR_NULL_POINTER;
    if (sp < 0 || M <= 0 || K <= 0 || N <= 0 || (K % BK) != 0 || M > 0x7fffffffLL || (reinterpret_cast<uintptr_t>(x) & 15))
        return TF_MSDA_ERR_BAD_DIMS;
    hipStream_t s = static_cast<hipStream_t>(stream);
    return with_scheme(sp, [&](auto spc) { return linear_split_sp<decltype(spc)::value>(x, w, bias, res, y, (int)M, K, N, relu, s); });
}

template <int SP>
int conv_launch_sp(const float *x, const Weight &w, const float *bias, float *out, const Conv3Args &ca, long long M, unsigned gz, int relu,
                   hipStream_t s)
{
    auto launch = [&](auto kern, unsigned bn) {
        const dim3 grid((unsigned)((M + 63) / 64), (unsigned)((ca.cout + bn - 1) / bn), gz);
        hipLaunchKernelGGL(kern, grid, dim3(THREADS), 0, s, x, w.p[0], w.p[1], w.p[2], w.scale, bias, out, ca);
    };
    if (ca.cout >= 128) {
        relu ? launch(split_conv3_kernel<SP, 64, 128, true>, 128) : launch(split_conv3_kernel<SP, 64, 128, false>, 128);
    } else {
        relu ? launch(split_conv3_kernel<SP, 64, 64, true>, 64) : launch(split_conv3_kernel<SP, 64, 64, false>, 64);
    }
    return hipGetLastError() == hipSuccess ? TF_MSDA_OK : TF_MSDA_ERR_LAUNCH;
}

int conv_split_impl(const float *x, const void *w_hi, const void *w_mid, const void *w_lo, const float *w_scale, const float *bias,
                    float *y, int nimg, int hin, int win, int cin, int cout, int stride, int ks, int relu, void *stream, int ksplit = 1,
                    float *workspace = nullptr)
{
    if (!x || !y) return TF_MSDA_ERR_NULL_POINTER;
    Weight w;
    const int sp = weight_scheme(w_hi, w_mid, w_lo, w_scale, w);
    if (sp == 0) return TF_MSDA_ERR_NULL_POINTER;
    if (sp < 0 || nimg <= 0 || hin <= 0 || win <= 0 || cin <= 0 || cout <= 0 || (cin % BK) != 0 || (stride != 1 && stride != 2) ||
        (reinterpret_cast<uintptr_t>(x) & 15))
        return TF_MSDA_ERR_BAD_DIMS;
    const int pad = ks == 3 ? 1 : 0;
    Conv3Args ca{nimg, hin, win, cin, (hin + 2 * pad - ks) / stride + 1, (win + 2 * pad - ks) / stride + 1, cout, stride, ks, pad, 0};
    const long long M = (long long)nimg * ca.hout * ca.wout;
    if (M <= 0 || (M + 256) * cout * 4 >= 0xC0000000LL || (long long)nimg * hin * win * cin * 4 >= 0xC0000000LL ||
        (long long)cout * ks * ks * cin * 2 >= 0xC0000000LL)
        return TF_MSDA_ERR_BAD_DIMS;
    hipStream_t s = static_cast<hipStream_t>(stream);
    const int slices = ks * ks * cin / BK;
    unsigned gz = 1;
    float *out = y;
    const float *kbias = bias;
    int krelu = relu;
    if (ksplit > 1) {
        if ((cout & 3) || (reinterpret_cast<uintptr_t>(workspace) | reinterpret_cast<uintptr_t>(y) | reinterpret_cast<uintptr_t>(bias)) & 15)
            return TF_MSDA_ERR_BAD_DIMS;
        ca.kslices = (slices + ksplit - 1) / ksplit;
        gz = (unsigned)((slices + ca.kslices - 1) / ca.kslices);
        out = workspace;
        kbias = nullptr;
        krelu = 0;
    }
    const int rc = with_scheme(sp, [&](auto spc) { return conv_launch_sp<decltype(spc)::value>(x, w, kbias, out, ca, M, gz, krelu, s); });
    if (rc != TF_MSDA_OK) return rc;
    if (ksplit > 1) {
        const long long mn4 = M * cout / 4;
        hipLaunchKernelGGL(conv_splitk_reduce_kernel, dim3((unsigned)((mn4 + 255) / 256)), dim3(256), 0, s, workspace, bias, y, mn4,
                           cout / 4, (int)gz, relu);
        if (hipGetLastError() != hipSuccess) return TF_MSDA_ERR_LAUNCH;
    }
    return TF_MSDA_OK;
}

}

extern "C" int tf_linear_split_f32(const float *x, const void *w_hi, const void *w_mid, const void *w_lo, const float *w_scale,
                                   const float *bias, float *y, int64_t M, int K, int N, int relu, void *stream)
{
    return linear_split_impl(x, w_hi, w_mid, w_lo, w_scale, bias, nullptr, y, M, K, N, relu, stream);
}

extern "C" int tf_linear_split_res_f32(const float *x, const void *w_hi, const void *w_mid, const void *w_lo, const float *w_scale,
                                       const float *bias, const float *residual, float *y, int64_t M, int K, int N, int relu, void *stream)
{
    if (!residual) return TF_MSDA_ERR_NULL_POINTER;
    return linear_split_impl(x, w_hi, w_mid, w_lo, w_scale, bias, residual, y, M, K, N, relu, stream);
}

extern "C" int tf_linear_split_add_f32(const float *x, const float *x2, const void *w_hi, const void *w_mid, const void *w_lo,
                                       const float *w_scale, const float *bias, float *y, int64_t M, int K, int N, void *stream)
{
    if (!x || !x2 || !y) return TF_MSDA_ERR_NULL_POINTER;
    Weight w;
    const int sp = weight_scheme(w_hi, w_mid, w_lo, w_scale, w);
    if (sp == 0) return TF_MSDA_ERR_NULL_POINTER;
    if (sp < 0 || M <= 0 || K <= 0 || N <= 0 || (K % BK) != 0 || M > 0x7fffffffLL ||
        ((reinterpret_cast<uintptr_t>(x) | reinterpret_cast<uintptr_t>(x2)) & 15))
        return TF_MSDA_ERR_BAD_DIMS;
    hipStream_t s = static_cast<hipStream_t>(stream);
    return with_scheme(sp, [&](auto spc) {
        constexpr int SP = decltype(spc)::value;
        if (M <= 4096) return launch_add<SP, 64, 64, true>(x, x2, w, bias, y, (int)M, K, N, s);
        if (N > 256 && N < 512) return launch_add<SP, 64, 128, false>(x, x2, w, bias, y, (int)M, K, N, s);
        return launch_add<SP, 64, 128, true>(x, x2, w, bias, y, (int)M, K, N, s);
    });
}

extern "C" int tf_conv3x3_splitk_f32(const float *x, const void *w_hi, const void *w_mid, const void *w_lo, const float *w_scale,
                                     const float *bias, float *y, float *workspace, int ksplit, int nimg, int hin, int win, int cin,
                                     int cout, int stride, int relu, void *stream)
{
    if (ksplit > 1 && !workspace) return TF_MSDA_ERR_NULL_POINTER;
    if (ksplit < 1 || ksplit > 64) return TF_MSDA_ERR_BAD_DIMS;
    return conv_split_impl(x, w_hi, w_mid, w_lo, w_scale, bias, y, nimg, hin, win, cin, cout, stride, 3, relu, stream, ksplit, workspace);
}

extern "C" int tf_conv1x1_splitk_f32(const float *x, const void *w_hi, const void *w_mid, const void *w_lo, const float *w_scale,
                                     const float *bias, float *y, float *workspace, int ksplit, int nimg, int hin, int win, int cin,
                                     int cout, int stride, int relu, void *stream)
{
    if (ksplit > 1 && !workspace) return TF_MSDA_ERR_NULL_POINTER;
    if (ksplit < 1 || ksplit > 64) return TF_MSDA_ERR_BAD_DIMS;
    return conv_split_impl(x, w_hi, w_mid, w_lo, w_scale, bias, y, nimg, hin, win, cin, cout, stride, 1, relu, stream, ksplit, workspace);
}

extern "C" int tf_conv3x3_split_f32(const float *x, const void *w_hi, const void *w_mid, const void *w_lo, const float *w_scale,
                                    const float *bias, float *y, int nimg, int hin, int win, int cin, int cout, int stride, int relu,
                                    void *stream)
{
    return conv_split_impl(x, w_hi, w_mid, w_lo, w_scale, bias, y, nimg, hin, win, cin, cout, stride, 3, relu, stream);
}

extern "C" int tf_conv1x1_strided_split_f32(const float *x, const void *w_hi, const void *w_mid, const void *w_lo, const float *w_scale,
                                            const float *bias, float *y, int nimg, int hin, int win, int cin, int cout, int stride,
                                            int relu, void *stream)
{
    return conv_split_impl(x, w_hi, w_mid, w_lo, w_scale, bias, y, nimg, hin, win, cin, cout, stride, 1, relu, stream);
}
```

trackformer_amd/deformable_transformer.py:

```python
import copy
import math

import torch
import torch.nn.functional as F
from torch import nn
from torch.nn.init import constant_, normal_, xavier_uniform_

from . import fused
from .msda import MSDeformAttn, attach_host_shapes
from .nested import inverse_sigmoid, is_all_valid


def _inference(module) -> bool:
    return (not module.training) and (not torch.is_grad_enabled())


def _ffn_hidden(linear, activation, x, inference):
    if inference and activation is F.relu and x.is_cuda and x.dtype == torch.float32:
        if fused.split_linear_enabled():
            y = fused.linear(x, linear.weight, linear.bias, relu=True)
            if y is not None:
                return y
        x2 = x.reshape(-1, x.shape[-1])
        y = torch._addmm_activation(linear.bias, x2, linear.weight.t(), use_gelu=False)
# ... 157 lines not shown
        cache = self.__dict__.setdefault("_ref_points_cache", {})
        hit = cache.get(key)
        if hit is None:
            value = lin(query_embed).sigmoid()
            if (query_embed.is_cuda and torch.cuda.is_current_stream_capturing()) or len(cache) >= _KEEP_CACHE_ENTRIES:
                return value
            hit = (value, query_param)
            if value.is_cuda:
                fused._publish_barrier(value.device)
            cache[key] = hit
        return hit[0]

    def _level_position_embedding(self, pos_embeds):
        def compute():
            return torch.cat([p.flatten(2).transpose(1, 2) + self.level_embed[lvl].view(1, 1, -1)
                              for lvl, p in enumerate(pos_embeds)], 1)
        if self.training or torch.is_grad_enabled():
            return compute()
        if not all(getattr(p, "_tf_cached_geometry", False) for p in pos_embeds):
            return compute()
        key = tuple((id(p), p._version) for p in pos_embeds) + (self.level_embed._version, self.level_embed.data_ptr())
        cache = self.__dict__.setdefault("_lvl_pos_cache", {})
        hit = cache.get(key)
        if hit is None:
            if (pos_embeds[0].is_cuda and torch.cuda.is_current_stream_capturing()) or len(cache) >= _KEEP_CACHE_ENTRIES:
                return compute()
            hit = (compute(), list(pos_embeds))
            if pos_embeds[0].is_cuda:
                fused._publish_barrier(pos_embeds[0].device)
            cache[key] = hit
        return hit[0]

    def forward(self, srcs, masks, pos_embeds, query_embed=None, targets=None):
        return self.decode(self.encode(srcs, masks, pos_embeds), query_embed, targets)

    def encode(self, srcs, masks, pos_embeds):
        shapes = tuple((int(s.shape[2]), int(s.shape[3])) for s in srcs)
        device = srcs[0].device
        src_flatten = torch.cat([s.flatten(2).transpose(1, 2) for s in srcs], 1)
        lvl_pos_embed_flatten = self._level_position_embedding(pos_embeds)
        unpadded = all(is_all_valid(m) for m in masks)
        if unpadded:
            mask_flatten = None
            valid_ratios = _GEOMETRY.unit_valid_ratios(src_flatten.shape[0], len(shapes), device)
        else:
            mask_flatten = torch.cat([m.flatten(1) for m in masks], 1)
            valid_ratios = torch.stack([self.get_valid_ratio(m) for m in masks], 1)
        spatial_shapes = _GEOMETRY.spatial_shapes(shapes, device)

        if self.multi_frame_attention_separate_encoder:
            half_t = src_flatten.shape[1] // 2
            half_l = self.num_feature_levels // 2

            def run(sl_t, sl_l):
                return self.encoder(
                    src_flatten[:, sl_t], _GEOMETRY.spatial_shapes(shapes[sl_l], device),
                    valid_ratios[:, sl_l], lvl_pos_embed_flatten[:, sl_t],
                    None if mask_flatten is None else mask_flatten[:, sl_t], unit_ratios=unpadded)
            prev_memory = run(slice(0, half_t), slice(0, half_l))
            memory = run(slice(half_t, None), slice(half_l, None))
            memory = torch.cat([memory, prev_memory], 1)
        else:
            memory = self.encoder(src_flatten, spatial_shapes, valid_ratios, lvl_pos_embed_flatten,
                                  mask_flatten, unit_ratios=unpadded)

        return {"memory": memory, "spatial_shapes": spatial_shapes, "valid_ratios": valid_ratios,
                "mask_flatten": mask_flatten, "device": device}

    def decode(self, enc, query_embed=None, targets=None):
        assert self.two_stage or query_embed is not None
        memory, spatial_shapes, valid_ratios = enc["memory"], enc["spatial_shapes"], enc["valid_ratios"]
        mask_flatten, device = enc["mask_flatten"], enc["device"]
        bs, _, c = memory.shape
        query_attn_mask = None
        filler_key_mask = None
        enc_outputs_class = enc_outputs_coord_unact = None
        if self.two_stage:
            pad = mask_flatten if mask_flatten is not None else \
                torch.zeros(memory.shape[:2], dtype=torch.bool, device=device)
            output_memory, output_proposals = self.gen_encoder_output_proposals(
                memory, pad, spatial_shapes)
            enc_outputs_class = self.decoder.class_embed[self.decoder.num_layers](output_memory)
            enc_outputs_coord_unact = \
                self.decoder.bbox_embed[self.decoder.num_layers](output_memory) + output_proposals
            topk = self.two_stage_num_proposals
            topk_proposals = torch.topk(enc_outputs_class[..., 0], topk, dim=1)[1]
            topk_coords_unact = torch.gather(
                enc_outputs_coord_unact, 1, topk_proposals.unsqueeze(-1).repeat(1, 1, 4)).detach()
            reference_points = topk_coords_unact.sigmoid()
            init_reference_out = reference_points
            pos_trans_out = self.pos_trans_norm(
                self.pos_trans(self.get_proposal_pos_embed(topk_coords_unact)))
            query_embed, tgt = torch.split(pos_trans_out, c, dim=2)
        else:
            query_param = query_embed
            query_embed, tgt = torch.split(query_embed, c, dim=1)
            query_embed = query_embed.unsqueeze(0).expand(bs, -1, -1)
            tgt = tgt.unsqueeze(0).expand(bs, -1, -1)
            reference_points = self._object_reference_points(query_param, query_embed, bs)

            if targets is not None and 'track_query_hs_embeds' in targets[0]:
                prev_hs_embed = torch.stack([t['track_query_hs_embeds'] for t in targets])
                prev_boxes = torch.stack([t['track_query_boxes'] for t in targets])
                query_embed = torch.cat([torch.zeros_like(prev_hs_embed), query_embed], dim=1)
                tgt = torch.cat([prev_hs_embed, tgt], dim=1)
                reference_points = torch.cat([prev_boxes[..., :2], reference_points], dim=1)
                if 'track_query_filler' in targets[0]:
                    filler = torch.stack([t['track_query_filler'] for t in targets])
                    filler_key_mask = torch.cat(
                        [filler, torch.zeros((bs, tgt.shape[1] - filler.shape[1]), dtype=torch.bool,
                                             device=filler.device)], dim=1)
            init_reference_out = reference_points

        hs, inter_references = self.decoder(tgt, reference_points, memory, spatial_shapes,
                                            valid_ratios, query_embed, mask_flatten,
                                            query_attn_mask, filler_key_mask)
        if self.two_stage:
            return (hs, memory, init_reference_out, inter_references, enc_outputs_class,
                    enc_outputs_coord_unact)
        return hs, memory, init_reference_out, inter_references, None, None


class DeformableTransformerEncoderLayer(nn.Module):
    def __init__(self, d_model=256, d_ffn=1024, dropout=0.1, activation="relu", n_levels=4,
                 n_heads=8, n_points=4):
        super().__init__()
        self.self_attn = MSDeformAttn(d_model, n_levels, n_heads, n_points)
        self.dropout1 = nn.Dropout(dropout)
        self.norm1 = nn.LayerNorm(d_model)
        self.linear1 = nn.Linear(d_model, d_ffn)
        self.activation = _get_activation_fn(activation)
        self.dropout2 = nn.Dropout(dropout)
        self.linear2 = nn.Linear(d_ffn, d_model)
        self.dropout3 = nn.Dropout(dropout)
        self.norm2 = nn.LayerNorm(d_model)

    @staticmethod
    def with_pos_embed(tensor, pos):
        return tensor if pos is None else tensor + pos

    def forward_ffn(self, src):
        inf = _inference(self)
        if inf and fused.ffn_fused_enabled() and self.activation is F.relu:
            out = fused.ffn(src, self.linear1, self.linear2, self.norm2, residual=src)
            if out is not None:
                return out
        src2 = fused.module_linear(self.linear2, self.dropout2(_ffn_hidden(self.linear1, self.activation, src, inf)), inf)
        return fused.residual_norm(src, self.dropout3(src2), self.norm2, inf)

    def forward(self, src, pos, reference_points, spatial_shapes, padding_mask=None):
        inf = _inference(self)
        q, q_pos = (src, pos) if (inf and pos is not None and fused.pos_add_fused_enabled()) else (self.with_pos_embed(src, pos), None)
        if inf and fused.linear_ln_fused_enabled():
            src = self.self_attn(q, reference_points, src, spatial_shapes, padding_mask,
                                 residual_norm=(src, self.norm1), query_pos=q_pos)
            return self.forward_ffn(src)
        src2 = self.self_attn(q, reference_points, src, spatial_shapes, padding_mask, query_pos=q_pos)
        src = fused.residual_norm(src, self.dropout1(src2), self.norm1, _inference(self))
        return self.forward_ffn(src)


class DeformableTransformerEncoder(nn.Module):
    def __init__(self, encoder_layer, num_layers):
        super().__init__()
        self.layers = _get_clones(encoder_layer, num_layers)
        self.num_layers = num_layers

    @staticmethod
    def get_reference_points(spatial_shapes, valid_ratios, device):
        if torch.is_tensor(spatial_shapes):
            spatial_shapes = _host_shapes(spatial_shapes)
        per_level = []
        for lvl, (h, w) in enumerate(spatial_shapes):
            ys = torch.linspace(0.5, h - 0.5, h, dtype=torch.float32, device=device)
            xs = torch.linspace(0.5, w - 0.5, w, dtype=torch.float32, device=device)
            ref_y, ref_x = torch.meshgrid(ys, xs, indexing="ij")
            ref_y = ref_y.reshape(-1)[None] / (valid_ratios[:, None, lvl, 1] * h)
            ref_x = ref_x.reshape(-1)[None] / (valid_ratios[:, None, lvl, 0] * w)
            per_level.append(torch.stack((ref_x, ref_y), -1))
        reference_points = torch.cat(per_level, 1)
        return reference_points[:, :, None] * valid_ratios[:, None]

    def forward(self, src, spatial_shapes, valid_ratios, pos=None, padding_mask=None,
                unit_ratios=False):
        reference_points = _GEOMETRY.encoder_reference_points(
            _host_shapes(spatial_shapes), valid_ratios, unit_ratios)
        output = src
        for layer in self.layers:
            output = layer(output, pos, reference_points, spatial_shapes, padding_mask)
        return output


class DeformableTransformerDecoderLayer(nn.Module):
    def __init__(self, d_model=256, d_ffn=1024, dropout=0.1, activation="relu", n_levels=4,
                 n_heads=8, n_points=4):
        super().__init__()
        self.cross_attn = MSDeformAttn(d_model, n_levels, n_heads, n_points)
        self.dropout1 = nn.Dropout(dropout)
        self.norm1 = nn.LayerNorm(d_model)
        self.self_attn = nn.MultiheadAttention(d_model, n_heads, dropout=dropout)
        self.dropout2 = nn.Dropout(dropout)
        self.norm2 = nn.LayerNorm(d_model)
        self.linear1 = nn.Linear(d_model, d_ffn)
        self.activation = _get_activation_fn(activation)
        self.dropout3 = nn.Dropout(dropout)
        self.linear2 = nn.Linear(d_ffn, d_model)
        self.dropout4 = nn.Dropout(dropout)
        self.norm3 = nn.LayerNorm(d_model)

    @staticmethod
    def with_pos_embed(tensor, pos):
        return tensor if pos is None else tensor + pos

    def forward_ffn(self, tgt):
        inf = _inference(self)
        if inf and fused.ffn_fused_enabled() and self.activation is F.relu:
            out = fused.ffn(tgt, self.linear1, self.linear2, self.norm3, residual=tgt)
            if out is not None:
                return out
        tgt2 = fused.module_linear(self.linear2, self.dropout3(_ffn_hidden(self.linear1, self.activation, tgt, inf)), inf)
        return fused.residual_norm(tgt, self.dropout4(tgt2), self.norm3, inf)

    def _self_attention_inference(self, qk_in, v_in, key_padding_mask, residual_norm=None, qk_pos=None):
        mha = self.self_attn
        E, H = mha.embed_dim, mha.num_heads
        w, b = mha.in_proj_weight, mha.in_proj_bias
        n, lq, _ = qk_in.shape
        qk = None
        if qk_pos is not None:
            qk = fused.linear_add(qk_in, qk_pos, w, b[:2 * E], rows=(0, 2 * E))
            if qk is None:
                qk_in = qk_in + qk_pos
        if qk is None:
            qk = fused.linear(qk_in, w, b[:2 * E], rows=(0, 2 * E))
        if qk is None:
            qk = F.linear(qk_in, w[:2 * E], b[:2 * E])
        v = fused.linear(v_in, w, b[2 * E:], rows=(2 * E, 3 * E))
        if v is None:
            v = F.linear(v_in, w[2 * E:], b[2 * E:])
        o = fused.mha_core(qk, v, H, key_padding_mask)
        if o is not None:
            if residual_norm is not None and fused.linear_ln_fused_enabled():
                y = fused.linear_residual_norm(o, mha.out_proj, residual_norm[0], residual_norm[1])
                if y is not None:
                    return y, True
            return fused.module_linear(mha.out_proj, o, True), False
        qk = qk.view(n, lq, 2, H, E // H)
        v = v.view(n, lq, H, E // H)
        q, k = qk[:, :, 0].transpose(1, 2), qk[:, :, 1].transpose(1, 2)
        mask = None
        if key_padding_mask is not None:
            mask = ~key_padding_mask[:, None, None, :]
        o = F.scaled_dot_product_attention(q, k, v.transpose(1, 2), attn_mask=mask)
        return mha.out_proj(o.transpose(1, 2).reshape(n, lq, E)), False

    def forward(self, tgt, query_pos, reference_points, src, src_spatial_shapes,
                src_padding_mask=None, query_attn_mask=None, filler_key_mask=None):
        key_mask = query_attn_mask if query_attn_mask is not None else filler_key_mask
        if _inference(self) and tgt.is_cuda and self.self_attn.in_proj_weight is not None:
            if query_pos is not None and fused.pos_add_fused_enabled():
                tgt2, normed = self._self_attention_inference(tgt, tgt, key_mask, residual_norm=(tgt, self.norm2), qk_pos=query_pos)
            else:
                tgt2, normed = self._self_attention_inference(self.with_pos_embed(tgt, query_pos), tgt, key_mask,
                                                              residual_norm=(tgt, self.norm2))
        else:
            normed = False
            q = k = self.with_pos_embed(tgt, query_pos)
            tgt2 = self.self_attn(q.transpose(0, 1), k.transpose(0, 1), tgt.transpose(0, 1),
                                  key_padding_mask=key_mask)[0].transpose(0, 1)
        tgt = tgt2 if normed else fused.residual_norm(tgt, self.dropout2(tgt2), self.norm2, _inference(self))
        inf = _inference(self)
        cq, cq_pos = (tgt, query_pos) if (inf and query_pos is not None and fused.pos_add_fused_enabled()) \
            else (self.with_pos_embed(tgt, query_pos), None)
        if inf and fused.linear_ln_fused_enabled():
            tgt = self.cross_attn(cq, reference_points, src, src_spatial_shapes, src_padding_mask, query_attn_mask,
                                  residual_norm=(tgt, self.norm1), query_pos=cq_pos)
            return self.forward_ffn(tgt)
        tgt2 = self.cross_attn(cq, reference_points, src, src_spatial_shapes, src_padding_mask, query_attn_mask,
                               query_pos=cq_pos)
        tgt = fused.residual_norm(tgt, self.dropout1(tgt2), self.norm1, _inference(self))
        return self.forward_ffn(tgt)


class DeformableTransformerDecoder(nn.Module):
    def __init__(self, decoder_layer, num_layers, return_intermediate=False):
        super().__init__()
        self.layers = _get_clones(decoder_layer, num_layers)
        self.num_layers = num_layers
        self.return_intermediate = return_intermediate
        self.bbox_embed = None
        self.class_embed = None

    def forward(self, tgt, reference_points, src, src_spatial_shapes, src_valid_ratios,
                query_pos=None, src_padding_mask=None, query_attn_mask=None, filler_key_mask=None):
        output = tgt
        intermediate = []
        intermediate_reference_points = []
        unit = getattr(src_valid_ratios, "_tf_unit", False)
        for lid, layer in enumerate(self.layers):
            if unit:
                reference_points_input = reference_points[:, :, None].expand(-1, -1, src_valid_ratios.shape[1], -1)
            elif reference_points.shape[-1] == 4:
                reference_points_input = reference_points[:, :, None] \
                    * torch.cat([src_valid_ratios, src_valid_ratios], -1)[:, None]
            else:
                assert reference_points.shape[-1] == 2
                reference_points_input = reference_points[:, :, None] * src_valid_ratios[:, None]
            output = layer(output, query_pos, reference_points_input, src, src_spatial_shapes,
                           src_padding_mask, query_attn_mask, filler_key_mask)
# ... 49 lines not shown
```

trackformer_amd/fused.py:

```python
import os
import threading

import torch
import torch.nn.functional as F

from . import _cabi


def _stream(device):
    return torch.cuda.current_stream(device).cuda_stream


def _param_ok(t, x):
    return (t.device == x.device and t.dtype == torch.float32 and t.is_contiguous()
            and t.data_ptr() % 16 == 0)


def bias_act_(x, bias, residual=None, relu=True):
    if not (x.is_cuda and x.dtype == torch.float32 and x.dim() == 4
            and x.is_contiguous(memory_format=torch.channels_last)):
        return None
    C = x.shape[1]
    if C % 4 or not _param_ok(bias, x) or x.data_ptr() % 16:
        return None
# ... 201 lines not shown
        if not (0 <= rows[0] < rows[1] <= N):
            return None
        N = rows[1] - rows[0]
    if x.shape[-1] != K or K % 32 or x.numel() == 0:
        return None
    if bias is not None and not (bias.dtype == torch.float32 and bias.is_contiguous() and bias.numel() == N
                                 and bias.device == x.device):
        return None
    x2 = x.reshape(-1, K)
    if not x2.is_contiguous():
        x2 = x2.contiguous()
    if residual is not None and not (residual.dtype == torch.float32 and residual.is_contiguous() and residual.device == x.device
                                     and residual.numel() == x2.shape[0] * N):
        return None
    if _use_packed(x2.shape[0], K, N) and not (x2.data_ptr() & 15) and (x2.shape[0] + 256) * N * 4 < 0xC0000000:
        packed = _packed_weight(weight, rows)
        if packed is not None:
            with torch.cuda.device(x.device):
                y = torch.empty((x2.shape[0], N), dtype=torch.float32, device=x.device)
                rc = _cabi.lib().tf_linear_packed_f32(x2.data_ptr(), packed.data_ptr(),
                                                      0 if bias is None else bias.data_ptr(), _ptr(residual), y.data_ptr(),
                                                      x2.shape[0], K, N, 1 if relu else 0, _terms(), _stream(x.device))
            _cabi.check(rc, "tf_linear_packed_f32")
            return y.view(*x.shape[:-1], N)
    pieces = _split_weight(weight)
    if rows is not None:
        pieces = _rows_of(pieces, rows)
    hi, mid, lo, wsc = pieces
    if (x2.data_ptr() | hi.data_ptr() | mid.data_ptr() | _ptr(lo)) & 15:
        return None
    with torch.cuda.device(x.device):
        y = torch.empty((x2.shape[0], N), dtype=torch.float32, device=x.device)
        if residual is None:
            rc = _cabi.lib().tf_linear_split_f32(x2.data_ptr(), hi.data_ptr(), mid.data_ptr(), _ptr(lo), _ptr(wsc),
                                                 0 if bias is None else bias.data_ptr(), y.data_ptr(), x2.shape[0], K, N,
                                                 1 if relu else 0, _stream(x.device))
        else:
            rc = _cabi.lib().tf_linear_split_res_f32(x2.data_ptr(), hi.data_ptr(), mid.data_ptr(), _ptr(lo), _ptr(wsc),
                                                     0 if bias is None else bias.data_ptr(), residual.data_ptr(),
                                                     y.data_ptr(), x2.shape[0], K, N, 1 if relu else 0, _stream(x.device))
    _cabi.check(rc, "tf_linear_split_f32")
    return y.view(*x.shape[:-1], N)


_ffn_fused = os.environ.get("TF_FFN_FUSED", "1") != "0"
_FFN_FUSED_MIN_ROWS = int(os.environ.get("TF_FFN_FUSED_MIN_ROWS", "4096"))


def ffn_fused_enabled():
    return _ffn_fused


def set_ffn_fused(on):
    global _ffn_fused
    prev, _ffn_fused = _ffn_fused, bool(on)
    return prev


def ffn(x, linear1, linear2, norm=None, residual=None):
    if not (_ffn_fused and _split_linear and x.is_cuda and x.dtype == torch.float32):
        return None
    w1, w2 = linear1.weight, linear2.weight
    F_, D = w1.shape
    if D not in (256, 288) or x.shape[-1] != D or tuple(w2.shape) != (D, F_) or F_ % 16 or F_ < 128 or x.numel() == 0:
        return None
    if not all(w.dtype == torch.float32 and w.is_contiguous() and w.device == x.device for w in (w1, w2)):
        return None
    x2 = x.reshape(-1, D)
    if not x2.is_contiguous():
        x2 = x2.contiguous()
    M = x2.shape[0]
    if M < _FFN_FUSED_MIN_ROWS or (M + 128) * D * 4 > 0xFFFFFFFF:
        return None
    vecs = [linear1.bias, linear2.bias]
    if norm is not None:
        if not (norm.elementwise_affine and tuple(norm.normalized_shape) == (D,)):
            return None
        vecs += [norm.weight, norm.bias]
    if not all(v is None or _param_ok(v, x) for v in vecs):
        return None
    if residual is not None:
        if residual.dtype != torch.float32 or residual.device != x.device or residual.numel() != x2.numel():
            return None
        residual = residual.reshape(-1, D)
        if not residual.is_contiguous():
            residual = residual.contiguous()
    if (x2.data_ptr() | (0 if residual is None else residual.data_ptr())) & 15:
        return None
    p1, p2 = _packed_weight(w1, None), _packed_weight(w2, None)
    if p1 is None or p2 is None:
        return None
    ptr = lambda t: 0 if t is None else t.data_ptr()
    with torch.cuda.device(x.device):
        y = torch.empty((M, D), dtype=torch.float32, device=x.device)
        rc = _cabi.lib().tf_ffn_fused_f32(x2.data_ptr(), p1.data_ptr(), ptr(linear1.bias), p2.data_ptr(), ptr(linear2.bias),
                                          ptr(residual), 0 if norm is None else norm.weight.data_ptr(),
                                          0 if norm is None else norm.bias.data_ptr(), 0.0 if norm is None else float(norm.eps),
                                          y.data_ptr(), M, D, F_, _terms(), _stream(x.device))
    _cabi.check(rc, "tf_ffn_fused_f32")
    return y.view(x.shape)


_linln_fused = os.environ.get("TF_LINLN_FUSED", "1") != "0"
_LINLN_MIN_ROWS = int(os.environ.get("TF_LINLN_MIN_ROWS", "256"))


def linear_ln_fused_enabled():
    return _linln_fused


def set_linear_ln_fused(on):
    global _linln_fused
    prev, _linln_fused = _linln_fused, bool(on)
    return prev


def linear_residual_norm(x, linear, residual, norm):
    if not (_linln_fused and _split_linear and x.is_cuda and x.dtype == torch.float32):
        return None
    w = linear.weight
    D = w.shape[0]
    if D not in (256, 288) or tuple(w.shape) != (D, D) or x.shape[-1] != D or x.numel() == 0:
        return None
    if not (w.dtype == torch.float32 and w.is_contiguous() and w.device == x.device
            and norm.elementwise_affine and tuple(norm.normalized_shape) == (D,)):
        return None
    x2 = x.reshape(-1, D)
    if not x2.is_contiguous():
        x2 = x2.contiguous()
    M = x2.shape[0]
    if M < _LINLN_MIN_ROWS or (M + 128) * D * 4 > 0xFFFFFFFF:
        return None
    if not all(v is None or _param_ok(v, x) for v in (linear.bias, norm.weight, norm.bias)):
        return None
    if residual.dtype != torch.float32 or residual.device != x.device or residual.numel() != x2.numel():
        return None
    residual = residual.reshape(-1, D)
    if not residual.is_contiguous():
        residual = residual.contiguous()
    if (x2.data_ptr() | residual.data_ptr()) & 15:
        return None
    packed = _packed_weight(w, None)
    if packed is None:
        return None
    with torch.cuda.device(x.device):
        y = torch.empty((M, D), dtype=torch.float32, device=x.device)
        rc = _cabi.lib().tf_linear_res_ln_f32(x2.data_ptr(), packed.data_ptr(), 0 if linear.bias is None else linear.bias.data_ptr(),
                                              residual.data_ptr(), norm.weight.data_ptr(), norm.bias.data_ptr(), float(norm.eps),
                                              y.data_ptr(), M, D, D, _terms(), _stream(x.device))
    _cabi.check(rc, "tf_linear_res_ln_f32")
    return y.view(x.shape)


_stem_pool_fused = os.environ.get("TF_STEM_POOL_FUSED", "1") != "0"


def stem_pool_fused_enabled():
    return _stem_pool_fused


def set_stem_pool_fused(on):
    global _stem_pool_fused
    prev, _stem_pool_fused = _stem_pool_fused, bool(on)
    return prev


_stem_conv_split = os.environ.get("TF_STEM_CONV_SPLIT", "1") != "0"


def stem_conv_split_enabled():
    return _stem_conv_split


def set_stem_conv_split(on):
    global _stem_conv_split
    prev, _stem_conv_split = _stem_conv_split, bool(on)
    return prev


def _stem_packed(weight):
    hit = getattr(weight, "_tf_stem_packed", None)
    terms = _terms()
    if hit is None or hit[0] != (weight._version, terms):
        if torch.cuda.is_current_stream_capturing():
            return None
        w = weight.detach()
        w2 = torch.zeros((64, 176), dtype=torch.float32, device=w.device)
        w2[:, :168] = F.pad(w, (0, 1)).reshape(64, 168)
        nbytes = _cabi.lib().tf_linear_packed_bytes(176, 64, terms)
        with torch.cuda.device(w.device):
            packed = torch.empty(nbytes, dtype=torch.uint8, device=w.device)
            rc = _cabi.lib().tf_linear_pack_weight_f32(w2.data_ptr(), packed.data_ptr(), 176, 64, terms, _stream(w.device))
        _cabi.check(rc, "tf_linear_pack_weight_f32")
        _publish_barrier(w.device)
        hit = ((weight._version, terms), packed)
        weight._tf_stem_packed = hit
    return hit[1]


def stem_conv(x, weight, bias=None, relu=False):
    if not (_stem_conv_split and _split_linear and x.is_cuda and x.dtype == torch.float32 and x.dim() == 4 and x.shape[1] == 3
            and tuple(weight.shape) == (64, 3, 7, 7) and weight.dtype == torch.float32 and weight.device == x.device
            and x.numel() > 0):
        return None
    if bias is not None and not (_param_ok(bias, x) and bias.numel() == 64):
        return None
    x = x if x.is_contiguous() else x.contiguous()
    n, _, h, w = x.shape
    ho, wo = (h - 1) // 2 + 1, (w - 1) // 2 + 1
    if n > 65535 or n * ho * wo * 256 >= 0xC0000000 or n * 3 * h * w >= 2 ** 31:
        return None
    packed = _stem_packed(weight)
    if packed is None:
        return None
    with torch.cuda.device(x.device):
        y = torch.empty((n, 64, ho, wo), dtype=torch.float32, device=x.device, memory_format=torch.channels_last)
        rc = _cabi.lib().tf_stem_conv7x7_f32(x.data_ptr(), packed.data_ptr(), 0 if bias is None else bias.data_ptr(), y.data_ptr(),
                                             n, h, w, 1 if relu else 0, _terms(), _stream(x.device))
    _cabi.check(rc, "tf_stem_conv7x7_f32")
    return y


def bias_relu_maxpool(x, bias):
    if not (x.is_cuda and x.dtype == torch.float32 and x.dim() == 4 and x.is_contiguous(memory_format=torch.channels_last)
            and x.numel() > 0 and x.shape[1] % 4 == 0 and _param_ok(bias, x) and bias.numel() == x.shape[1]
            and x.data_ptr() % 16 == 0):
        return None
    n, c, h, w = x.shape
    with torch.cuda.device(x.device):
        out = torch.empty((n, c, (h - 1) // 2 + 1, (w - 1) // 2 + 1), dtype=torch.float32, device=x.device,
                          memory_format=torch.channels_last)
        rc = _cabi.lib().tf_bias_relu_maxpool_f32(x.data_ptr(), bias.data_ptr(), out.data_ptr(), n, h, w, c, _stream(x.device))
    _cabi.check(rc, "tf_bias_relu_maxpool_f32")
    return out


_heads_split = os.environ.get("TF_HEADS_SPLIT", "1") != "0"


def heads_split_enabled():
    return _heads_split


def set_heads_split(on):
    global _heads_split
    prev, _heads_split = _heads_split, bool(on)
    return prev


def head_linear(module, x, relu=False):
    if _heads_split and not module.training and not torch.is_grad_enabled():
        y = linear(x, module.weight, module.bias, relu=relu)
        if y is not None:
            return y
    y = module(x)
    return F.relu(y) if relu else y


_pos_add_fused = os.environ.get("TF_POS_ADD_FUSED", "1") != "0"


def pos_add_fused_enabled():
    return _pos_add_fused


def set_pos_add_fused(on):
    global _pos_add_fused
    prev, _pos_add_fused = _pos_add_fused, bool(on)
    return prev


def linear_add(x, x2, weight, bias=None, rows=None):
    if not (_pos_add_fused and _split_linear and x.is_cuda and x.dtype == torch.float32 and x2.dtype == torch.float32
            and x2.shape == x.shape and x2.device == x.device and weight.dtype == torch.float32 and weight.dim() == 2
            and weight.is_contiguous() and weight.device == x.device):
        return None
    N, K = weight.shape
    if rows is not None:
        if not (0 <= rows[0] < rows[1] <= N):
            return None
        N = rows[1] - rows[0]
    if x.shape[-1] != K or K % 32 or x.numel() == 0:
        return None
    if bias is not None and not (bias.dtype == torch.float32 and bias.is_contiguous() and bias.numel() == N
                                 and bias.device == x.device):
        return None
    a, b = x.reshape(-1, K), x2.reshape(-1, K)
    a = a if a.is_contiguous() else a.contiguous()
    b = b if b.is_contiguous() else b.contiguous()
    pieces = _split_weight(weight)
    if rows is not None:
        pieces = _rows_of(pieces, rows)
    hi, mid, lo, wsc = pieces
    if (a.data_ptr() | b.data_ptr() | hi.data_ptr() | mid.data_ptr() | _ptr(lo)) & 15:
        return None
    with torch.cuda.device(x.device):
        y = torch.empty((a.shape[0], N), dtype=torch.float32, device=x.device)
        rc = _cabi.lib().tf_linear_split_add_f32(a.data_ptr(), b.data_ptr(), hi.data_ptr(), mid.data_ptr(), _ptr(lo), _ptr(wsc),
                                                 0 if bias is None else bias.data_ptr(), y.data_ptr(), a.shape[0], K, N,
                                                 _stream(x.device))
    _cabi.check(rc, "tf_linear_split_add_f32")
    return y.view(*x.shape[:-1], N)


def conv3x3(x, w_taps, bias, relu, stride):
    if not (_split_linear and x.is_cuda and x.dtype == torch.float32 and x.dim() == 4
            and x.is_contiguous(memory_format=torch.channels_last) and w_taps.dtype == torch.float32
            and w_taps.dim() == 2 and w_taps.is_contiguous() and w_taps.device == x.device):
        return None
    n, cin, h, w = x.shape
    cout = w_taps.shape[0]
    ks = 3 if w_taps.shape[1] == 9 * cin else 1
    if w_taps.shape[1] != ks * ks * cin or cin % 32 or stride not in (1, 2) or x.numel() == 0:
        return None
    if bias is not None and not (bias.dtype == torch.float32 and bias.is_contiguous() and bias.numel() == cout
                                 and bias.device == x.device):
        return None
    pad = 1 if ks == 3 else 0
    ho, wo = (h + 2 * pad - ks) // stride + 1, (w + 2 * pad - ks) // stride + 1
    cin_ok = cin % 64 == 0 or (ks == 3 and stride == 1 and _conv_halo and cin % 32 == 0)
    stream_route = (_conv_stream and _conv_stream_wins(n * ho * wo, cout) and cin_ok and not (x.data_ptr() & 15)
                    and n * h * w * cin * 4 < 0xC0000000 and (n * ho * wo + 256) * cout * 4 < 0xC0000000)
    halo = ks == 3 and stride == 1 and _conv_halo and stream_route
    ksplit = _conv_ksplit(n * ho * wo, ks * ks * cin, cout, _HALO_KSPLIT_POLICY if halo else None)
    if ks == 1 and (ksplit < _CONV1X1_MIN_PIECES or not _conv1x1_splitk):
        ksplit = 1
    if stream_route:
        packed = _packed_weight(w_taps, None)
        if packed is not None:
            with torch.cuda.device(x.device):
                y = torch.empty((n, ho, wo, cout), dtype=torch.float32, device=x.device)
                ws = torch.empty((ksplit, n * ho * wo * cout), dtype=torch.float32, device=x.device) if ksplit > 1 else None
                rc = _cabi.lib().tf_conv_packed_f32(x.data_ptr(), packed.data_ptr(), _ptr(bias), 0, y.data_ptr(), _ptr(ws), ksplit,
                                                    n, h, w, cin, cout, ks, stride, 1 if relu else 0, _terms(), _stream(x.device))
            _cabi.check(rc, "tf_conv_packed_f32")
            return y.permute(0, 3, 1, 2)
    if (n * h * w * cin * 4 >= 0xC0000000 or (n * ho * wo + 256) * cout * 4 >= 0xC0000000 or cout * ks * ks * cin * 2 >= 0xC0000000):
        return None
    hi, mid, lo, wsc = _split_weight(w_taps)
    if (x.data_ptr() | hi.data_ptr() | mid.data_ptr() | _ptr(lo)) & 15:
        return None
    with torch.cuda.device(x.device):
        y = torch.empty((n, ho, wo, cout), dtype=torch.float32, device=x.device)
        if ksplit > 1:
            ws = torch.empty((ksplit, n * ho * wo * cout), dtype=torch.float32, device=x.device)
            fn = _cabi.lib().tf_conv3x3_splitk_f32 if ks == 3 else _cabi.lib().tf_conv1x1_splitk_f32
            rc = fn(x.data_ptr(), hi.data_ptr(), mid.data_ptr(), _ptr(lo), _ptr(wsc), 0 if bias is None else bias.data_ptr(), y.data_ptr(),
                    ws.data_ptr(), ksplit, n, h, w, cin, cout, stride, 1 if relu else 0, _stream(x.device))
        else:
            fn = _cabi.lib().tf_conv3x3_split_f32 if ks == 3 else _cabi.lib().tf_conv1x1_strided_split_f32
            rc = fn(x.data_ptr(), hi.data_ptr(), mid.data_ptr(), _ptr(lo), _ptr(wsc), 0 if bias is None else bias.data_ptr(), y.data_ptr(),
                    n, h, w, cin, cout, stride, 1 if relu else 0, _stream(x.device))
    _cabi.check(rc, "tf_conv3x3_split_f32")
    return y.permute(0, 3, 1, 2)


_conv_splitk = os.environ.get("TF_CONV_SPLITK", "1") not in ("", "0")

_conv_stream = os.environ.get("TF_CONV_STREAM", "1") not in ("", "0")
_CONV_STREAM_ALL = os.environ.get("TF_CONV_STREAM") == "all"


def _conv_stream_wins(m, cout):
    return _CONV_STREAM_ALL or _terms() == 16 or (cout >= 128 and m >= 8192)


def set_conv_stream(on):
    global _conv_stream, _CONV_STREAM_ALL
    prev = "all" if (_conv_stream and _CONV_STREAM_ALL) else _conv_stream
    _conv_stream, _CONV_STREAM_ALL = bool(on), on == "all"
    return prev



_KSPLIT_POLICY = tuple(int(v) for v in os.environ.get("TF_CONV_KSPLIT_POLICY", "768,300,8,32").split(","))


def set_conv_ksplit_policy(target_blocks, leave_alone_blocks, min_slices_per_piece, min_slices):
    global _KSPLIT_POLICY
    prev, _KSPLIT_POLICY = _KSPLIT_POLICY, (int(target_blocks), int(leave_alone_blocks), int(min_slices_per_piece), int(min_slices))
    return prev


def conv1x1_wants_split_k(m, cin, cout):
    return _conv1x1_splitk and _conv_ksplit(m, cin, cout) >= _CONV1X1_MIN_PIECES


_conv1x1_splitk = os.environ.get("TF_CONV1X1_SPLITK", "1") not in ("", "0")
_CONV1X1_MIN_PIECES = 3


def set_conv1x1_splitk(on):
    global _conv1x1_splitk
    prev, _conv1x1_splitk = _conv1x1_splitk, bool(on)
    return prev


_conv_halo = os.environ.get("TF_CONV_HALO", "1") not in ("", "0")
_HALO_KSPLIT_POLICY = tuple(int(v) for v in os.environ.get("TF_CONV_HALO_KSPLIT_POLICY", "512,300,9,32").split(","))


def set_conv_halo(on):
    global _conv_halo
    prev, _conv_halo = _conv_halo, bool(on)
    _cabi.lib().tf_msda_set_option(b"conv_halo", 1 if on else 0)
    return prev


def _conv_ksplit(m, k, cout, policy=None):
    if not _conv_splitk or cout % 4:
        return 1
    target, alone, per_piece, min_slices = policy or _KSPLIT_POLICY
    blocks = -(-m // 64) * -(-cout // (128 if cout >= 128 else 64))
    slices = k // 32
    if blocks >= alone or slices < min_slices:
        return 1
    return max(1, min(64, target // blocks, slices // per_piece))


_input_proj_fused = os.environ.get("TF_INPUT_PROJ_FUSED", "1") != "0"


def set_input_proj_fused(on):
    global _input_proj_fused
    prev, _input_proj_fused = _input_proj_fused, bool(on)
    return prev


def groupnorm_nhwc(x2, n_img, gn, relu=False):
    if not (x2.is_cuda and x2.dtype == torch.float32 and x2.dim() == 2 and x2.is_contiguous()
            and gn.weight is not None and gn.bias is not None and _param_ok(gn.weight, x2) and _param_ok(gn.bias, x2)):
        return None
    rows, c = x2.shape
    if rows % n_img or c != gn.num_channels or c % 4 or c > 1024 or gn.num_groups > 256 or n_img > 65535 or (x2.data_ptr() & 15):
        return None
    hw = rows // n_img
    with torch.cuda.device(x2.device):
        out = torch.empty_like(x2)
        ws = torch.empty(2 * n_img * gn.num_groups, dtype=torch.float64, device=x2.device)
        fn = _cabi.lib().tf_groupnorm_relu_nhwc_f32 if relu else _cabi.lib().tf_groupnorm_nhwc_f32
        rc = fn(x2.data_ptr(), gn.weight.data_ptr(), gn.bias.data_ptr(), out.data_ptr(), ws.data_ptr(), n_img, hw, c, gn.num_groups,
                float(gn.eps), hw * c, hw * c, _stream(x2.device))
    _cabi.check(rc, "tf_groupnorm_nhwc_f32")
    return out


def mask_label_map(logits, order, pad_hw, img_hw, out_hw, threshold=0.5):
    if not (_postprocess_fused and logits.is_cuda and logits.dtype == torch.float32 and logits.dim() == 3 and logits.is_contiguous()
            and 0 < len(order) <= 32767 and logits.numel() > 0):
        return None
    n, h, w = logits.shape
    if any(r >= n for r in order) or img_hw[0] > pad_hw[0] or img_hw[1] > pad_hw[1]:
        return None
    with torch.cuda.device(logits.device):
        order_dev = torch.tensor(list(order), dtype=torch.int32).to(logits.device, non_blocking=True)
# ... 189 lines not shown
        y = linear(x, module.weight, module.bias)
        if y is not None:
            return y
    return module(x)


def mha_core(qk, v, num_heads, key_padding_mask=None):
    if os.environ.get("TF_NO_MHA") == "1":
        return None
    if not (qk.is_cuda and qk.dtype == torch.float32 and v.dtype == torch.float32 and v.device == qk.device
            and qk.dim() == 3 and v.dim() == 3 and qk.is_contiguous() and v.is_contiguous()):
        return None
    n, length, e2 = qk.shape
    e = e2 // 2
    if e2 != 2 * e or v.shape != (n, length, e) or e % num_heads:
        return None
    d = e // num_heads
    if d not in (16, 32, 36, 64) or e % 4 or length > 2300 or (qk.data_ptr() | v.data_ptr()) & 15 or (e * 4) % 16:
        return None
    mask_ptr = 0
    if key_padding_mask is not None:
        if (key_padding_mask.shape != (n, length) or key_padding_mask.device != qk.device
                or key_padding_mask.dtype not in (torch.bool, torch.uint8)):
            return None
        key_padding_mask = key_padding_mask.to(torch.uint8).contiguous()
        mask_ptr = key_padding_mask.data_ptr()
    with torch.cuda.device(qk.device):
        out = torch.empty((n, length, e), dtype=torch.float32, device=qk.device)
        q_ptr = qk.data_ptr()
        rc = _cabi.lib().tf_mha_core_f32(q_ptr, q_ptr + e * 4, v.data_ptr(), out.data_ptr(), mask_ptr, n, length, length,
                                         num_heads, d, e2, e2, e, e, float(d) ** -0.5, _stream(qk.device))
    if rc == -2:
        return None
    _cabi.check(rc, "tf_mha_core_f32")
    return out


import contextlib
import functools

F16_ACTIVATION_LIMIT = 65504.0 * 16.0
_check_finite = os.environ.get("TF_SPLIT_CHECK_FINITE", "0") not in ("", "0")
_n_six_term_routes = 0
_range_audit = None
_route_epoch = 0



def route_epoch():
    return _route_epoch


def debug_checks_active():
    return _check_finite or _range_audit is not None


def set_check_finite(on):
    global _check_finite, _route_epoch
    prev, _check_finite = _check_finite, bool(on)
    if prev != _check_finite:
        _route_epoch += 1
    return prev


def _routed(weight):
    return getattr(weight, "_tf_six_terms", False)


def route_six_terms(weight, on=True):
    global _n_six_term_routes, _route_epoch
    if bool(_routed(weight)) != bool(on):
        weight._tf_six_terms = bool(on)
        _n_six_term_routes += 1 if on else -1
        _route_epoch += 1


def inherit_route(new, *sources):
    if any(src is not None and _routed(src) for src in sources) and not _routed(new):
        route_six_terms(new)
    return new


def six_term_routes():
    return _n_six_term_routes


@contextlib.contextmanager
def audit_activation_range(route=True, safety=4.0):
    global _range_audit, _route_epoch
    report = {"limit": F16_ACTIVATION_LIMIT, "safety": safety, "largest": 0.0, "layers": [], "routed": 0}
    prev, _range_audit = _range_audit, {}
    _route_epoch += 1
    try:
        yield report
    finally:
        seen, _range_audit = _range_audit, prev
        _route_epoch += 1
        for (name, _ids), (ws, shapes, amax) in sorted(seen.items(), key=lambda kv: -kv[1][2]):
            report["layers"].append((name, shapes, amax))
            report["largest"] = max(report["largest"], amax)
            if route and not (amax * safety < F16_ACTIVATION_LIMIT):
                for w in ws:
                    route_six_terms(w)
                report["routed"] += 1


def _amax(t):
    return float(t.detach().abs().max()) if t is not None and t.numel() else 0.0


def _ranged(name, weights_of, acts_of):
    def deco(fn):
        @functools.wraps(fn)
        def wrapped(*a, **k):
            if _split_terms != 16 or not (_n_six_term_routes or _check_finite or _range_audit is not None):
                return fn(*a, **k)
            ws = [w for w in weights_of(*a, **k) if w is not None]
            checks = _check_finite or _range_audit is not None
            if checks and ws and ws[0].is_cuda and torch.cuda.is_current_stream_capturing():
                raise RuntimeError("fused.%s: an activation-range audit / the finite check (set_check_finite, TF_SPLIT_CHECK_FINITE) "
                                   "reads results on the host and cannot run while a HIP graph is being captured -- run the model "
                                   "eagerly under them (GraphedDetector does so by itself), then capture" % name)
            route6 = any(_routed(w) for w in ws)
            if route6:
                _tls.terms = 6
            try:
                y = fn(*a, **k)
            finally:
                if route6:
                    _tls.terms = None
            if y is None:
                return y
            if _range_audit is not None:
                key = (name, tuple(id(w) for w in ws))
                rec = _range_audit.setdefault(key, [ws, tuple(tuple(w.shape) for w in ws), 0.0])
                rec[2] = max(rec[2], max(_amax(t) for t in acts_of(*a, **k)))
            if _check_finite and not bool(torch.isfinite(y).all()):
                raise FloatingPointError(
                    "%s produced a non-finite result (largest |input| %.3g; the fp16 split product represents activations up to "
                    "%.3g -- fused.audit_activation_range() routes such layers through the six-term product, "
                    "fused.set_split_terms(6) all of them)" % (name, max(_amax(t) for t in acts_of(*a, **k)), F16_ACTIVATION_LIMIT))
            return y
        return wrapped
    return deco


def _ffn_acts(x, linear1, linear2, norm=None, residual=None):
    hidden = F.relu(F.linear(x, linear1.weight, linear1.bias)) if _range_audit is not None else None
    return (x, hidden)


linear = _ranged("linear", lambda x, weight, *a, **k: (weight,), lambda x, *a, **k: (x,))(linear)
linear_add = _ranged("linear_add", lambda x, x2, weight, *a, **k: (weight,), lambda x, x2, *a, **k: (x + x2,))(linear_add)
ffn = _ranged("ffn", lambda x, linear1, linear2, *a, **k: (linear1.weight, linear2.weight), _ffn_acts)(ffn)
linear_residual_norm = _ranged("linear_residual_norm", lambda x, linear, *a, **k: (linear.weight,), lambda x, *a, **k: (x,))(linear_residual_norm)
stem_conv = _ranged("stem_conv", lambda x, weight, *a, **k: (weight,), lambda x, *a, **k: (x,))(stem_conv)
conv3x3 = _ranged("conv3x3", lambda x, w_taps, *a, **k: (w_taps,), lambda x, *a, **k: (x,))(conv3x3)
```

trackformer_amd/msda.py:

```python
import ctypes
import math

import torch
import torch.nn.functional as F
from torch import nn
from torch.autograd import Function
from torch.autograd.function import once_differentiable
from torch.nn.init import constant_, xavier_uniform_

from . import _cabi, fused

import os as _os

FUSED_INFERENCE = _os.environ.get("TF_MSDA_FUSED", "1") != "0"

_HOST_SHAPE_ATTR = "_tf_msda_host_shapes"
_shape_array_cache = {}


def attach_host_shapes(spatial_shapes, host_shapes):
    setattr(spatial_shapes, _HOST_SHAPE_ATTR, tuple((int(h), int(w)) for h, w in host_shapes))
    return spatial_shapes


# ... 110 lines not shown
    grad_output = grad_output.contiguous()
    lib = _cabi.lib()
    if not value.is_cuda:
        grad_value, grad_loc, grad_attn = torch.empty_like(value), torch.empty_like(sampling_loc), torch.empty_like(attn_weight)
        shp = _host_shape_tensor(spatial_shapes)
        rc = getattr(lib, "tf_msda_backward_host_" + suf)(
            value.data_ptr(), shp.data_ptr(), sampling_loc.data_ptr(), attn_weight.data_ptr(), grad_output.data_ptr(),
            grad_value.data_ptr(), grad_loc.data_ptr(), grad_attn.data_ptr(), N, S, M, D, L, Lq, P)
        _cabi.check(rc, "ms_deform_attn_backward")
        return [grad_value, grad_loc, grad_attn]
    with torch.cuda.device(value.device):
        grad_value = torch.empty_like(value)
        grad_loc = torch.empty_like(sampling_loc)
        grad_attn = torch.empty_like(attn_weight)
        tail, shp, keep = _shape_args(spatial_shapes, value)
        stream = torch.cuda.current_stream().cuda_stream
        rc = getattr(lib, "tf_msda_backward_%s%s" % (suf, tail))(
            value.data_ptr(), shp, sampling_loc.data_ptr(), attn_weight.data_ptr(),
            grad_output.data_ptr(), grad_value.data_ptr(), grad_loc.data_ptr(),
            grad_attn.data_ptr(), N, S, M, D, L, Lq, P, stream)
    del keep
    _cabi.check(rc, "ms_deform_attn_backward")
    return [grad_value, grad_loc, grad_attn]


def ms_deform_attn_forward_fused(value, spatial_shapes, reference_points, qproj, n_heads, n_levels,
                                 n_points):
    hs = _host_shapes_of(spatial_shapes)
    if hs is None:
        raise RuntimeError("ms_deform_attn_forward_fused needs host-side level shapes "
                           "(attach_host_shapes)")
    if value.dim() != 4 or qproj.dim() != 3 or reference_points.dim() != 4:
        raise RuntimeError("ms_deform_attn_forward_fused: expected value[N,S,M,D], reference_points[N,Lq,L,2|4], "
                           "qproj[N,Lq,3*M*L*P]")
    for name, t in (("value", value), ("reference_points", reference_points), ("qproj", qproj)):
        if t.dtype != torch.float32:
            raise RuntimeError("ms_deform_attn_forward_fused: %s must be float32, got %s" % (name, t.dtype))
        if not t.is_cuda or t.device != value.device:
            raise RuntimeError("ms_deform_attn_forward_fused: %s must be a CUDA tensor on value's device" % name)
    if not value.is_contiguous():
        raise RuntimeError("ms_deform_attn_forward_fused: value tensor has to be contiguous")
    N, S, M, D = value.shape
    Lq = qproj.shape[1]
    L, P = n_levels, n_points
    if M != n_heads or qproj.shape[-1] != 3 * M * L * P or qproj.shape[0] != N \
            or tuple(reference_points.shape[:3]) != (N, Lq, L):
        raise RuntimeError("ms_deform_attn_forward_fused: inconsistent tensor shapes")
    reference_points = reference_points.contiguous()
    ld = qproj.stride(1)
    if not (Lq > 1 and qproj.stride(2) == 1 and (N == 1 or qproj.stride(0) == Lq * ld) and ld >= qproj.shape[-1]
            and ld % 2 == 0 and qproj.data_ptr() % 8 == 0):
        qproj = qproj.contiguous()
        ld = qproj.shape[-1]
    lib = _cabi.lib()
    with torch.cuda.device(value.device):
        out = torch.empty((N, Lq, M * D), dtype=value.dtype, device=value.device)
        arr = _shape_array(hs)
        rc = lib.tf_msda_forward_fused_f32(
            value.data_ptr(), ctypes.cast(arr, ctypes.c_void_p), reference_points.data_ptr(),
            reference_points.shape[-1], qproj.data_ptr(), ld, 0, 2 * M * L * P,
            out.data_ptr(), N, S, M, D, L, Lq, P, torch.cuda.current_stream().cuda_stream)
    _cabi.check(rc, "ms_deform_attn_forward_fused")
    return out


class _CatProjection:

    def __init__(self):
        self.key = None
        self.weight = None
        self.bias = None

    def get(self, mod):
        srcs = (mod.sampling_offsets.weight, mod.sampling_offsets.bias,
                mod.attention_weights.weight, mod.attention_weights.bias)
        key = tuple((t.data_ptr(), t._version, t.device, t.dtype) for t in srcs)
        if key != self.key:
            with torch.no_grad():
                self.weight = torch.cat([srcs[0], srcs[2]], 0).contiguous()
                self.bias = torch.cat([srcs[1], srcs[3]], 0).contiguous()
            self.key = key
        return self.weight, self.bias


class MSDeformAttnFunction(Function):

    @staticmethod
    def forward(ctx, value, value_spatial_shapes, sampling_locations, attention_weights,
                im2col_step):
        ctx.im2col_step = im2col_step
        ctx.host_shapes = _host_shapes_of(value_spatial_shapes)
        output = ms_deform_attn_forward(value, value_spatial_shapes, sampling_locations,
                                        attention_weights, ctx.im2col_step)
        ctx.save_for_backward(value, value_spatial_shapes, sampling_locations, attention_weights)
        return output

    @staticmethod
    @once_differentiable
    def backward(ctx, grad_output):
        value, value_spatial_shapes, sampling_locations, attention_weights = ctx.saved_tensors
        if ctx.host_shapes is not None:
            attach_host_shapes(value_spatial_shapes, ctx.host_shapes)
        grad_value, grad_sampling_loc, grad_attn_weight = ms_deform_attn_backward(
            value, value_spatial_shapes, sampling_locations, attention_weights, grad_output,
            ctx.im2col_step)
        return grad_value, None, grad_sampling_loc, grad_attn_weight, None


class _Normed:
    __slots__ = ("value",)

    def __init__(self, value):
        self.value = value


class MSDeformAttn(nn.Module):

    def __init__(self, d_model=256, n_levels=4, n_heads=8, n_points=4, im2col_step=64):
        super().__init__()
        if d_model % n_heads != 0:
            raise ValueError("d_model must be divisible by n_heads, got %d and %d" %
                             (d_model, n_heads))
        self.im2col_step = im2col_step
        self.d_model = d_model
        self.n_levels = n_levels
        self.n_heads = n_heads
        self.n_points = n_points

        self.sampling_offsets = nn.Linear(d_model, n_heads * n_levels * n_points * 2)
        self.attention_weights = nn.Linear(d_model, n_heads * n_levels * n_points)
        self.value_proj = nn.Linear(d_model, d_model)
        self.output_proj = nn.Linear(d_model, d_model)
        self._cat_proj = _CatProjection()
        self._reset_parameters()

    def _reset_parameters(self):
        constant_(self.sampling_offsets.weight.data, 0.)
        dirs = [(a, b) for a in (-1, 0, 1) for b in (-1, 0, 1) if (a, b) != (0, 0)]
        if self.n_heads != len(dirs):
            raise ValueError("MSDeformAttn bias initialisation requires n_heads == 8")
        grid = torch.tensor(dirs, dtype=torch.float32).view(self.n_heads, 1, 1, 2)
        grid = grid.repeat(1, self.n_levels, self.n_points, 1)
        scale = torch.arange(1, self.n_points + 1, dtype=torch.float32).view(1, 1, -1, 1)
        with torch.no_grad():
            self.sampling_offsets.bias = nn.Parameter((grid * scale).reshape(-1))
        constant_(self.attention_weights.weight.data, 0.)
        constant_(self.attention_weights.bias.data, 0.)
        xavier_uniform_(self.value_proj.weight.data)
        constant_(self.value_proj.bias.data, 0.)
        xavier_uniform_(self.output_proj.weight.data)
        constant_(self.output_proj.bias.data, 0.)

    def forward(self, query, reference_points, input_flatten, input_spatial_shapes,
                input_padding_mask=None, query_attn_mask=None, residual_norm=None, query_pos=None):
        if residual_norm is not None:
            out = self._forward(query, reference_points, input_flatten, input_spatial_shapes, input_padding_mask,
                                query_attn_mask, residual_norm, query_pos)
            if isinstance(out, _Normed):
                return out.value
            return fused.residual_norm(residual_norm[0], out, residual_norm[1], True)
        return self._forward(query, reference_points, input_flatten, input_spatial_shapes, input_padding_mask, query_attn_mask,
                             None, query_pos)

    def _forward(self, query, reference_points, input_flatten, input_spatial_shapes, input_padding_mask, query_attn_mask,
                 residual_norm, query_pos=None):
        N, Len_q, _ = query.shape
        N, Len_in, _ = input_flatten.shape
        hs = _host_shapes_of(input_spatial_shapes)
        if hs is not None:
            if sum(h * w for h, w in hs) != Len_in:
                raise AssertionError("sum of H_l*W_l does not match the flattened input length")
        else:
            assert (input_spatial_shapes[:, 0] * input_spatial_shapes[:, 1]).sum() == Len_in

        M, L, P = self.n_heads, self.n_levels, self.n_points
        inference = not self.training and not torch.is_grad_enabled()
        value = fused.module_linear(self.value_proj, input_flatten, inference)
        if input_padding_mask is not None:
            value = value.masked_fill(input_padding_mask[..., None], float(0))
        value = value.view(N, Len_in, M, self.d_model // M)

        if (FUSED_INFERENCE and hs is not None and query_attn_mask is None and value.is_cuda
                and value.dtype == torch.float32 and not self.training
                and not torch.is_grad_enabled() and reference_points.shape[-1] in (2, 4)
                and (self.d_model // M) % 4 == 0 and P in (1, 2, 4, 8)):
            w, b = self._cat_proj.get(self)
            qproj = None
            if query_pos is not None:
                qproj = fused.linear_add(query, query_pos, w, b)
                if qproj is None:
                    query = query + query_pos
            if qproj is None:
                qproj = fused.linear(query, w, b) if fused.split_linear_enabled() else None
            if qproj is None:
                qproj = F.linear(query, w, b)
            output = ms_deform_attn_forward_fused(value, input_spatial_shapes, reference_points,
                                                  qproj, M, L, P)
            if residual_norm is not None:
                y = fused.linear_residual_norm(output, self.output_proj, residual_norm[0], residual_norm[1])
                if y is not None:
                    return _Normed(y)
            return fused.module_linear(self.output_proj, output, True)

        if query_pos is not None:
            query = query + query_pos
        sampling_offsets = self.sampling_offsets(query).view(N, Len_q, M, L, P, 2)
        attention_weights = self.attention_weights(query).view(N, Len_q, M, L * P)
        attention_weights = F.softmax(attention_weights, -1).view(N, Len_q, M, L, P)
        if query_attn_mask is not None:
            attention_weights = attention_weights.masked_fill(
                query_attn_mask[..., None, None, None], float(0))

        if reference_points.shape[-1] == 2:
            sampling_locations = reference_points[:, :, None, :, None, :] \
                + sampling_offsets / input_spatial_shapes[None, None, None, :, None, :]
        elif reference_points.shape[-1] == 4:
            sampling_locations = reference_points[:, :, None, :, None, :2] \
                + sampling_offsets / P * reference_points[:, :, None, :, None, 2:] * 0.5
        else:
            raise ValueError('Last dim of reference_points must be 2 or 4, but get {} instead.'
                             .format(reference_points.shape[-1]))
        output = MSDeformAttnFunction.apply(value, input_spatial_shapes, sampling_locations,
                                            attention_weights, self.im2col_step)
        return self.output_proj(output)
```

Measured before the change: 386.8.

## Fuse encoder value/query projections and output-proj+LN with FFN kernel

Adds a merged split-fp16 linear kernel that computes the value projection from the source and the sampling-offset/attention-weight projection from source+pos in a single pass, sharing the activation read. It also adds a kernel that runs output projection, residual add and LayerNorm, then the FFN and a second LayerNorm, all in one launch, keeping the intermediate row tile in LDS. This removes launches and HBM round trips of the encoder-layer intermediates. In exchange the kernels get more complex, with larger register and LDS pressure, and the merged path only engages above a row threshold.

New measurement: 343.2. -11.3%, worse.

```diff
diff --git a/include/tf_fused.h b/include/tf_fused.h
--- a/include/tf_fused.h
+++ b/include/tf_fused.h
@@ -64,6 +64,11 @@
 int tf_linear_split_add_f32(const float *x, const float *x2, const void *w_hi, const void *w_mid, const void *w_lo, const float *w_scale,
                             const float *bias, float *y, int64_t M, int K, int N, void *stream);
 
+int tf_linear_split_add2_f32(const float *x, const float *x2, const void *wv_hi, const void *wv_mid, const void *wv_lo,
+                             const float *wv_scale, const float *bias_v, float *value, int Nv, const void *wq_hi, const void *wq_mid,
+                             const void *wq_lo, const float *wq_scale, const float *bias_q, float *qproj, int Nq, int64_t M, int K,
+                             void *stream);
+
 int64_t tf_linear_packed_bytes(int K, int N, int terms);
 int tf_linear_pack_weight_f32(const float *w, void *packed, int K, int N, int terms, void *stream);
 int tf_linear_packed_f32(const float *x, const void *w_packed, const float *bias, const float *residual, float *y, int64_t M, int K,
@@ -80,6 +85,11 @@
                      const float *residual, const float *ln_weight, const float *ln_bias, float ln_eps, float *y, int64_t M,
                      int d_model, int d_ffn, int terms, void *stream);
 
+int tf_attn_ffn_fused_f32(const float *attn, const void *wo_packed, const float *bo, const float *residual, const float *ln1_weight,
+                          const float *ln1_bias, float ln1_eps, const void *w1_packed, const float *b1, const void *w2_packed,
+                          const float *b2, const float *ln2_weight, const float *ln2_bias, float ln2_eps, float *y, int64_t M,
+                          int d_model, int d_ffn, int terms, void *stream);
+
 int tf_mha_core_f32(const float *q, const float *k, const float *v, float *out, const unsigned char *key_mask,
                     int N, int Lq, int Lk, int H, int D, int ldq, int ldk, int ldv, int ldo, float scale,
                     void *stream);
diff --git a/trackformer_amd/_cabi.py b/trackformer_amd/_cabi.py
--- a/trackformer_amd/_cabi.py
+++ b/trackformer_amd/_cabi.py
@@ -48,6 +48,8 @@
     "tf_linear_pack_weight_f32",
     "tf_linear_packed_f32",
     "tf_linear_split_add_f32",
+    "tf_linear_split_add2_f32",
+    "tf_attn_ffn_fused_f32",
     "tf_ffn_fused_f32",
     "tf_linear_res_ln_f32",
     "tf_conv_packed_f32",
@@ -155,6 +157,10 @@
     L.tf_ffn_fused_f32.argtypes = [vp, vp, vp, vp, vp, vp, vp, vp, ctypes.c_float, vp, ctypes.c_int64, ci, ci, ci, vp]
     L.tf_linear_split_add_f32.restype = ci
     L.tf_linear_split_add_f32.argtypes = [vp, vp, vp, vp, vp, vp, vp, vp, ctypes.c_int64, ci, ci, vp]
+    L.tf_linear_split_add2_f32.restype = ci
+    L.tf_linear_split_add2_f32.argtypes = [vp] * 8 + [ci] + [vp] * 6 + [ci, ctypes.c_int64, ci, vp]
+    L.tf_attn_ffn_fused_f32.restype = ci
+    L.tf_attn_ffn_fused_f32.argtypes = [vp] * 6 + [ctypes.c_float] + [vp] * 6 + [ctypes.c_float, vp, ctypes.c_int64, ci, ci, ci, vp]
     L.tf_linear_packed_f32.restype = ci
     L.tf_linear_packed_f32.argtypes = [vp, vp, vp, vp, vp, ctypes.c_int64, ci, ci, ci, ci, vp]
     L.tf_conv_packed_f32.restype = ci
diff --git a/trackformer_amd/build.py b/trackformer_amd/build.py
--- a/trackformer_amd/build.py
+++ b/trackformer_amd/build.py
@@ -83,7 +83,7 @@
     out_dir = os.path.join(REPO_DIR, "tools", "bin")
     lib = os.path.join(LIB_DIR, "libtf_msda.so")
     built = []
-    for name in ("msda_bench", "linear_bench", "ffn_bench"):
+    for name in ("msda_bench", "linear_bench", "ffn_bench", "enc_layer_bench"):
         src = os.path.join(REPO_DIR, "tools", name + ".cpp")
         if not os.path.exists(src):
             continue
diff --git a/trackformer_amd/csrc/ffn_fused.hip b/trackformer_amd/csrc/ffn_fused.hip
--- a/trackformer_amd/csrc/ffn_fused.hip
+++ b/trackformer_amd/csrc/ffn_fused.hip
@@ -157,11 +157,20 @@
                                                        (unsigned)((m0 + i * 32 + frow) * D + cbase + 32 * j + 8 * g) * 4u, 0, tfm::kStoreAux);
 }
 
-template <int SP, int D, int TI, bool LN>
-__global__ void __launch_bounds__(Geo<D>::NT, 1)
-ffn_fused_kernel(const float *__restrict__ X, const u32x4 *__restrict__ W1p, const float *__restrict__ b1,
-                 const u32x4 *__restrict__ W2p, const float *__restrict__ b2, const float *R,
-                 const float *__restrict__ gamma, const float *__restrict__ beta, float eps, float *Y, int M, int F)
+struct AttnHead {
+    const float *A;
+    const u32x4 *Wop;
+    const float *bo;
+    const float *R0;
+    const float *gamma, *beta;
+    float eps;
+};
+
+template <int SP, int D, int TI, bool LN, bool ATTN>
+__device__ __forceinline__ void
+ffn_block(const float *__restrict__ X, const u32x4 *__restrict__ W1p, const float *__restrict__ b1,
+          const u32x4 *__restrict__ W2p, const float *__restrict__ b2, const float *R,
+          const float *__restrict__ gamma, const float *__restrict__ beta, float eps, float *Y, int M, int F, const AttnHead &ah)
 {
     using G = Geo<D>;
     constexpr int BM = TI * 32, TJ = G::TJ, NW = G::NW, XS = G::XS, HS = G::HS, RING = G::RING, UPC = G::UPC, U1 = G::U1, U2 = G::U2;
@@ -191,19 +200,6 @@
                 for (int p = 0; p < NB; ++p) dst[j * NB + p] = W2p[(((size_t)(TJ * wave + j) * KQ2 + q) * NB + p) * 64 + lane];
         }
     };
-    static_for<G::AHEAD>([&](auto uc) { load_unit(0, uc, ring[decltype(uc)::value]); });
-    __builtin_amdgcn_sched_barrier(0);
-    stage_rows<SP, D, TI>(X, M, m0, sX, tid);
-    __syncthreads();
-
-    f32x16 accy[TI][TJ];
-#pragma unroll
-    for (int i = 0; i < TI; ++i)
-#pragma unroll
-        for (int j = 0; j < TJ; ++j)
-#pragma unroll
-            for (int e = 0; e < 16; ++e) accy[i][j][e] = 0.f;
-
     const float *const r1 = reinterpret_cast<const float *>(W1p + (size_t)ntiles1 * G::KQ1 * NB * 64);
     const float *const r2 = reinterpret_cast<const float *>(W2p + (size_t)((D + 255) / 256 * 8) * KQ2 * NB * 64);
     const int frow = (lane & 31), fk = (lane >> 5) * 8;
@@ -216,6 +212,95 @@
     const __amdgpu_buffer_rsrc_t rrs = __builtin_amdgcn_make_buffer_rsrc(const_cast<float *>(R ? R : X), 0, R ? bytes : 0u, 0x00020000);
     const int cbase = wave * (32 * TJ) + 4 * (lane >> 5);
     f32x4 v[TI][TJ][4];
+    f32x16 accy[TI][TJ];
+    auto clear_accy = [&]() {
+#pragma unroll
+        for (int i = 0; i < TI; ++i)
+#pragma unroll
+            for (int j = 0; j < TJ; ++j)
+#pragma unroll
+                for (int e = 0; e < 16; ++e) accy[i][j][e] = 0.f;
+    };
+
+    if constexpr (!ATTN) {
+        static_for<G::AHEAD>([&](auto uc) { load_unit(0, uc, ring[decltype(uc)::value]); });
+        __builtin_amdgcn_sched_barrier(0);
+        stage_rows<SP, D, TI>(X, M, m0, sX, tid);
+        __syncthreads();
+    } else {
+        constexpr int KQ = G::KQ1;
+        const int lane1 = __lane_id(), frow1 = lane1 & 31, cbase1 = wave * (32 * TJ) + 4 * (lane1 >> 5);
+        static_assert(NB * TJ <= US && G::AHEAD <= KQ, "an output-projection unit fits a ring slot");
+        auto load_o = [&](auto uc, u32x4 (&dst)[US]) {
+            constexpr int u = decltype(uc)::value;
+#pragma unroll
+            for (int j = 0; j < TJ; ++j)
+#pragma unroll
+                for (int p = 0; p < NB; ++p) dst[j * NB + p] = ah.Wop[(((size_t)(TJ * wave + j) * KQ + u) * NB + p) * 64 + lane];
+        };
+        static_for<G::AHEAD>([&](auto uc) { load_o(uc, ring[decltype(uc)::value % RING]); });
+        __builtin_amdgcn_sched_barrier(0);
+        stage_rows<SP, D, TI>(ah.A, M, m0, sX, tid);
+        __syncthreads();
+        clear_accy();
+        const __amdgpu_buffer_rsrc_t bors =
+            __builtin_amdgcn_make_buffer_rsrc(const_cast<float *>(ah.bo ? ah.bo : ah.A), 0, ah.bo ? (unsigned)D * 4u : 0u, 0x00020000);
+        const __amdgpu_buffer_rsrc_t r0rs = __builtin_amdgcn_make_buffer_rsrc(const_cast<float *>(ah.R0), 0, bytes, 0x00020000);
+        u32x4 af[2][TI][NA];
+        f32x4 x1[TI][TJ][4];
+        auto read_a = [&](auto stc) {
+            constexpr int st = decltype(stc)::value;
+#pragma unroll
+            for (int i = 0; i < TI; ++i)
+#pragma unroll
+                for (int p = 0; p < NA; ++p)
+                    af[st & 1][i][p] = *reinterpret_cast<const u32x4 *>(&sX[(p * BM + i * 32) * XS + xoff + st * 16]);
+        };
+        read_a(std::integral_constant<int, 0>{});
+        static_for<KQ>([&](auto stc) {
+            constexpr int st = decltype(stc)::value, ahead = st + G::AHEAD;
+            if constexpr (ahead < KQ) load_o(std::integral_constant<int, ahead>{}, ring[ahead % RING]);
+            if constexpr (st == KQ - G::AHEAD) {
+#pragma unroll
+                for (int i = 0; i < TI; ++i)
+#pragma unroll
+                    for (int j = 0; j < TJ; ++j)
+#pragma unroll
+                        for (int g = 0; g < 4; ++g)
+                            x1[i][j][g] = __builtin_bit_cast(f32x4, __builtin_amdgcn_raw_buffer_load_b128(
+                                                                       r0rs, (unsigned)((m0 + i * 32 + frow1) * D + cbase1 + 32 * j + 8 * g) * 4u, 0, 0));
+            }
+            if constexpr (st + 1 < KQ) read_a(std::integral_constant<int, st + 1>{});
+            __builtin_amdgcn_sched_barrier(0);
+            const u32x4 (&cur)[US] = ring[st % RING];
+            u32x4 wf[TJ][NB];
+#pragma unroll
+            for (int j = 0; j < TJ; ++j)
+#pragma unroll
+                for (int p = 0; p < NB; ++p) wf[j][p] = cur[j * NB + p];
+            mfma_tiles<SP, TI, TJ, false>(accy, af[st & 1], wf);
+        });
+        __builtin_amdgcn_sched_barrier(0);
+        static_for<G::AHEAD>([&](auto uc) { load_unit(0, uc, ring[decltype(uc)::value]); });
+        __builtin_amdgcn_sched_barrier(0);
+        const float *const ro = reinterpret_cast<const float *>(ah.Wop + (size_t)((D + 255) / 256 * 8) * KQ * NB * 64);
+        rows_epilogue<D, TI, true, F16>(accy, x1, bors, ro, ah.gamma, ah.beta, ah.eps, yrs, reinterpret_cast<float *>(sH), m0, wave, lane1);
+#pragma unroll
+        for (int i = 0; i < TI; ++i)
+#pragma unroll
+            for (int j = 0; j < TJ; ++j)
+#pragma unroll
+                for (int g = 0; g < 4; ++g) {
+                    u32x2 pc[NA];
+                    split4<SP>(x1[i][j][g], pc);
+#pragma unroll
+                    for (int p = 0; p < NA; ++p)
+                        *reinterpret_cast<u32x2 *>(&sX[(p * BM + i * 32 + frow1) * XS + cbase1 + 32 * j + 8 * g]) = pc[p];
+                }
+        __builtin_amdgcn_s_waitcnt(0x0F70);
+        __syncthreads();
+    }
+    clear_accy();
 
     for (int c = 0; c < nchunks; ++c) {
         const int cn = min(c + 1, nchunks - 1);
@@ -319,6 +404,24 @@
     rows_epilogue<D, TI, LN, F16>(accy, v, b2rs, r2, gamma, beta, eps, yrs, reinterpret_cast<float *>(sH), m0, wave, lane);
 }
 
+template <int SP, int D, int TI, bool LN>
+__global__ void __launch_bounds__(Geo<D>::NT, 1)
+ffn_fused_kernel(const float *__restrict__ X, const u32x4 *__restrict__ W1p, const float *__restrict__ b1,
+                 const u32x4 *__restrict__ W2p, const float *__restrict__ b2, const float *R,
+                 const float *__restrict__ gamma, const float *__restrict__ beta, float eps, float *Y, int M, int F)
+{
+    ffn_block<SP, D, TI, LN, false>(X, W1p, b1, W2p, b2, R, gamma, beta, eps, Y, M, F, AttnHead{});
+}
+
+template <int SP, int D, int TI>
+__global__ void __launch_bounds__(Geo<D>::NT, 1)
+attn_ffn_fused_kernel(const AttnHead ah, const u32x4 *__restrict__ W1p, const float *__restrict__ b1, const u32x4 *__restrict__ W2p,
+                      const float *__restrict__ b2, const float *__restrict__ gamma, const float *__restrict__ beta, float eps, float *Y,
+                      int M, int F)
+{
+    ffn_block<SP, D, TI, true, true>(ah.A, W1p, b1, W2p, b2, Y, gamma, beta, eps, Y, M, F, ah);
+}
+
 template <int SP, int D, int TI>
 int launch_ffn(const float *x, const u32x4 *w1, const float *b1, const u32x4 *w2, const float *b2, const float *res,
                const float *gamma, const float *beta, float eps, float *y, int M, int F, hipStream_t s)
@@ -337,6 +440,26 @@
     const int blocks = (M + 32 * TI - 1) / (32 * TI);
     void *argv[] = {(void *)&x, (void *)&w1, (void *)&b1, (void *)&w2, (void *)&b2, (void *)&res,
                     (void *)&gamma, (void *)&beta, (void *)&eps, (void *)&y, (void *)&M, (void *)&F};
+    return hipLaunchKernel(fn, dim3((unsigned)blocks), dim3(Geo<D>::NT), argv, lds, s) == hipSuccess ? TF_MSDA_OK : TF_MSDA_ERR_LAUNCH;
+}
+
+template <int SP, int D, int TI>
+int launch_attn_ffn(const AttnHead &ah, const u32x4 *w1, const float *b1, const u32x4 *w2, const float *b2, const float *gamma,
+                    const float *beta, float eps, float *y, int M, int F, hipStream_t s)
+{
+    constexpr size_t lds = ffn_lds_bytes<D>(TI, Split<SP>::NA);
+    static_assert(lds <= 160 * 1024, "the two tiles do not fit the LDS of a CU");
+    const void *fn = (const void *)&attn_ffn_fused_kernel<SP, D, TI>;
+    static std::atomic<unsigned> raised;
+    int dev = 0;
+    (void)hipGetDevice(&dev);
+    if (dev >= 32 || !(raised.load() & (1u << dev))) {
+        if (hipFuncSetAttribute(fn, hipFuncAttributeMaxDynamicSharedMemorySize, (int)lds) != hipSuccess) return TF_MSDA_ERR_LAUNCH;
+        if (dev < 32) raised.fetch_or(1u << dev);
+    }
+    const int blocks = (M + 32 * TI - 1) / (32 * TI);
+    void *argv[] = {(void *)&ah, (void *)&w1, (void *)&b1, (void *)&w2, (void *)&b2, (void *)&gamma, (void *)&beta, (void *)&eps,
+                    (void *)&y, (void *)&M, (void *)&F};
     return hipLaunchKernel(fn, dim3((unsigned)blocks), dim3(Geo<D>::NT), argv, lds, s) == hipSuccess ? TF_MSDA_OK : TF_MSDA_ERR_LAUNCH;
 }
 
@@ -558,6 +681,47 @@
     default:
         if constexpr (three_tiles) return launch_ffn<SP, D, 3>(x, w1, b1, w2, b2, residual, g, b, eps, y, M, F, s);
         else return launch_ffn<SP, D, 2>(x, w1, b1, w2, b2, residual, g, b, eps, y, M, F, s);
+    }
+}
+
+template <int SP, int D>
+int dispatch_attn_ffn(const AttnHead &ah, const u32x4 *w1, const float *b1, const u32x4 *w2, const float *b2, const float *g,
+                      const float *b, float eps, float *y, int M, int F, hipStream_t s)
+{
+    if (F < Geo<D>::CH || (F & 15)) return TF_MSDA_ERR_BAD_DIMS;
+    constexpr bool three_tiles = D == 256 && Split<SP>::NB == 2;
+    const int want = ffn_ti();
+    const bool ti2 = want == 2 || (want >= 3 && !three_tiles);
+    if (ti2 && tfm::ffn_tail_split()) {
+        const int cus = ffn_num_cus();
+        const long long per_round = 64LL * cus;
+        const int main_rows = (int)(M / per_round * per_round), rem = M - main_rows;
+        if (main_rows > 0 && rem > 0 && rem <= 32LL * cus) {
+            int rc = launch_attn_ffn<SP, D, 2>(ah, w1, b1, w2, b2, g, b, eps, y, main_rows, F, s);
+            if (rc != TF_MSDA_OK) return rc;
+            const size_t off = (size_t)main_rows * D;
+            AttnHead t = ah;
+            t.A += off;
+            t.R0 += off;
+            return launch_attn_ffn<SP, D, 1>(t, w1, b1, w2, b2, g, b, eps, y + off, rem, F, s);
+        }
+    }
+    switch (want) {
+    case 1: return launch_attn_ffn<SP, D, 1>(ah, w1, b1, w2, b2, g, b, eps, y, M, F, s);
+    case 2: return launch_attn_ffn<SP, D, 2>(ah, w1, b1, w2, b2, g, b, eps, y, M, F, s);
+    default:
+        if constexpr (three_tiles) return launch_attn_ffn<SP, D, 3>(ah, w1, b1, w2, b2, g, b, eps, y, M, F, s);
+        else return launch_attn_ffn<SP, D, 2>(ah, w1, b1, w2, b2, g, b, eps, y, M, F, s);
+    }
+}
+
+template <int D>
+int dispatch_attn_ffn_scheme(int sp, const AttnHead &ah, const u32x4 *w1, const float *b1, const u32x4 *w2, const float *b2,
+                             const float *g, const float *b, float eps, float *y, int M, int F, hipStream_t s)
+{
+    switch (sp) {
+    case 3: return dispatch_attn_ffn<3, D>(ah, w1, b1, w2, b2, g, b, eps, y, M, F, s);
+    default: return dispatch_attn_ffn<16, D>(ah, w1, b1, w2, b2, g, b, eps, y, M, F, s);
     }
 }
 
@@ -620,3 +784,28 @@
     return d_model == 256 ? dispatch_ffn_scheme<256>(sp, x, w1, b1, w2, b2, residual, ln_weight, ln_bias, ln_eps, y, (int)M, d_ffn, s)
                           : dispatch_ffn_scheme<288>(sp, x, w1, b1, w2, b2, residual, ln_weight, ln_bias, ln_eps, y, (int)M, d_ffn, s);
 }
+
+extern "C" int tf_attn_ffn_fused_f32(const float *attn, const void *wo_packed, const float *bo, const float *residual,
+                                     const float *ln1_weight, const float *ln1_bias, float ln1_eps, const void *w1_packed,
+                                     const float *b1, const void *w2_packed, const float *b2, const float *ln2_weight,
+                                     const float *ln2_bias, float ln2_eps, float *y, int64_t M, int d_model, int d_ffn, int terms,
+                                     void *stream)
+{
+    if (!attn || !wo_packed || !residual || !ln1_weight || !ln1_bias || !w1_packed || !w2_packed || !ln2_weight || !ln2_bias || !y)
+        return TF_MSDA_ERR_NULL_POINTER;
+    const int sp = split_scheme(terms);
+    if (M <= 0 || (d_model != 256 && d_model != 288) || d_ffn <= 0 || sp == 0 ||
+        (M + 128) * (int64_t)d_model * 4 > 0xFFFFFFFFLL)
+        return TF_MSDA_ERR_BAD_DIMS;
+    uintptr_t al = reinterpret_cast<uintptr_t>(attn) | reinterpret_cast<uintptr_t>(wo_packed) | reinterpret_cast<uintptr_t>(bo) |
+                   reinterpret_cast<uintptr_t>(residual) | reinterpret_cast<uintptr_t>(ln1_weight) | reinterpret_cast<uintptr_t>(ln1_bias) |
+                   reinterpret_cast<uintptr_t>(w1_packed) | reinterpret_cast<uintptr_t>(b1) | reinterpret_cast<uintptr_t>(w2_packed) |
+                   reinterpret_cast<uintptr_t>(b2) | reinterpret_cast<uintptr_t>(ln2_weight) | reinterpret_cast<uintptr_t>(ln2_bias) |
+                   reinterpret_cast<uintptr_t>(y);
+    if (al & 15) return TF_MSDA_ERR_BAD_DIMS;
+    const AttnHead ah{attn, static_cast<const u32x4 *>(wo_packed), bo, residual, ln1_weight, ln1_bias, ln1_eps};
+    const u32x4 *w1 = static_cast<const u32x4 *>(w1_packed), *w2 = static_cast<const u32x4 *>(w2_packed);
+    hipStream_t s = static_cast<hipStream_t>(stream);
+    return d_model == 256 ? dispatch_attn_ffn_scheme<256>(sp, ah, w1, b1, w2, b2, ln2_weight, ln2_bias, ln2_eps, y, (int)M, d_ffn, s)
+                          : dispatch_attn_ffn_scheme<288>(sp, ah, w1, b1, w2, b2, ln2_weight, ln2_bias, ln2_eps, y, (int)M, d_ffn, s);
+}
diff --git a/trackformer_amd/csrc/linear_split.hip b/trackformer_amd/csrc/linear_split.hip
--- a/trackformer_amd/csrc/linear_split.hip
+++ b/trackformer_amd/csrc/linear_split.hip
@@ -18,12 +18,18 @@
 
 __device__ __forceinline__ int stage_row(int q) { return (q & ~7) | ((q & 1) << 2) | ((q & 7) >> 1); }
 
+template <int SP, int BM, int BN>
+struct GemmTiles {
+    unsigned short a[Split<SP>::NA][BM * LDS_STRIDE];
+    unsigned short b[Split<SP>::NB][BN * LDS_STRIDE];
+};
+
 template <int SP, int BM, int BN, bool RELU, bool PREFETCH, bool RESID, bool BUFST, bool XADD = false>
 __device__ __forceinline__ void
-split_gemm_body(const float *__restrict__ X, const unsigned short *__restrict__ Whi,
+split_gemm_body(GemmTiles<SP, BM, BN> &tiles, const float *__restrict__ X, const unsigned short *__restrict__ Whi,
                 const unsigned short *__restrict__ Wmid, const unsigned short *__restrict__ Wlo, const float *__restrict__ Wsc,
                 const float *__restrict__ bias, const float *__restrict__ R, float *__restrict__ Y, int M, int K, int N,
-                const float *__restrict__ X2 = nullptr)
+                const float *__restrict__ X2 = nullptr, int bx = -1, int by = -1)
 {
     constexpr int NA = Split<SP>::NA, NB = Split<SP>::NB;
     constexpr bool F16 = Split<SP>::F16;
@@ -32,10 +38,10 @@
     constexpr int XV = (BM * BK / 4) / THREADS;
     constexpr int WV = (BN * BK / 8) / THREADS;
     static_assert(XV >= 1 && WV >= 1, "tile too small for 256 threads");
-    __shared__ __attribute__((aligned(16))) unsigned short sA[NA][BM * LDS_STRIDE];
-    __shared__ __attribute__((aligned(16))) unsigned short sB[NB][BN * LDS_STRIDE];
+    auto &sA = tiles.a;
+    auto &sB = tiles.b;
     const int tid = threadIdx.x, lane = tid & 63, wave = tid >> 6;
-    const int m0 = blockIdx.x * BM, n0 = blockIdx.y * BN;
+    const int m0 = (bx < 0 ? (int)blockIdx.x : bx) * BM, n0 = (by < 0 ? (int)blockIdx.y : by) * BN;
     const int wm = (wave >> 1) * (BM / 2), wn = (wave & 1) * (BN / 2);
 
     f32x16 acc[TI][TJ];
@@ -176,7 +182,8 @@
                   const unsigned short *__restrict__ Wmid, const unsigned short *__restrict__ Wlo, const float *__restrict__ Wsc,
                   const float *__restrict__ bias, float *__restrict__ Y, int M, int K, int N)
 {
-    split_gemm_body<SP, BM, BN, RELU, PREFETCH, false, BUFST>(X, Whi, Wmid, Wlo, Wsc, bias, nullptr, Y, M, K, N);
+    __shared__ __attribute__((aligned(16))) GemmTiles<SP, BM, BN> tiles;
+    split_gemm_body<SP, BM, BN, RELU, PREFETCH, false, BUFST>(tiles, X, Whi, Wmid, Wlo, Wsc, bias, nullptr, Y, M, K, N);
 }
 
 template <int SP, int BM, int BN, bool RELU, bool PREFETCH, bool BUFST = false>
@@ -185,7 +192,8 @@
                       const unsigned short *__restrict__ Wmid, const unsigned short *__restrict__ Wlo, const float *__restrict__ Wsc,
                       const float *__restrict__ bias, const float *__restrict__ R, float *__restrict__ Y, int M, int K, int N)
 {
-    split_gemm_body<SP, BM, BN, RELU, PREFETCH, true, BUFST>(X, Whi, Wmid, Wlo, Wsc, bias, R, Y, M, K, N);
+    __shared__ __attribute__((aligned(16))) GemmTiles<SP, BM, BN> tiles;
+    split_gemm_body<SP, BM, BN, RELU, PREFETCH, true, BUFST>(tiles, X, Whi, Wmid, Wlo, Wsc, bias, R, Y, M, K, N);
 }
 
 template <int SP, int BM, int BN, bool PREFETCH, bool BUFST>
@@ -194,7 +202,33 @@
                       const unsigned short *__restrict__ Wmid, const unsigned short *__restrict__ Wlo, const float *__restrict__ Wsc,
                       const float *__restrict__ bias, float *__restrict__ Y, int M, int K, int N)
 {
-    split_gemm_body<SP, BM, BN, false, PREFETCH, false, BUFST, true>(X, Whi, Wmid, Wlo, Wsc, bias, nullptr, Y, M, K, N, X2);
+    __shared__ __attribute__((aligned(16))) GemmTiles<SP, BM, BN> tiles;
+    split_gemm_body<SP, BM, BN, false, PREFETCH, false, BUFST, true>(tiles, X, Whi, Wmid, Wlo, Wsc, bias, nullptr, Y, M, K, N, X2);
+}
+
+struct Add2Out {
+    const unsigned short *w[3];
+    const float *scale, *bias;
+    float *y;
+    int n;
+};
+
+template <int SP, int BM, int BN, bool PREFETCH, bool BUFST>
+__global__ void __launch_bounds__(THREADS)
+split_gemm_add2_kernel(const float *__restrict__ X, const float *__restrict__ X2, const Add2Out v, const Add2Out q, int M, int K,
+                       int ntv, int ntiles)
+{
+    __shared__ __attribute__((aligned(16))) GemmTiles<SP, BM, BN> tiles;
+    const int g = blockIdx.x & 7, idx = blockIdx.x >> 3;
+    const int r = idx / ntiles, t = idx - r * ntiles;
+    const int rb = 8 * r + g;
+    if (rb * BM >= M) return;
+    if (t < ntv)
+        split_gemm_body<SP, BM, BN, false, PREFETCH, false, BUFST>(tiles, X, v.w[0], v.w[1], v.w[2], v.scale, v.bias, nullptr, v.y, M, K, v.n,
+                                                                   nullptr, rb, t);
+    else
+        split_gemm_body<SP, BM, BN, false, PREFETCH, false, BUFST, true>(tiles, X, q.w[0], q.w[1], q.w[2], q.scale, q.bias, nullptr, q.y, M, K,
+                                                                         q.n, X2, rb, t - ntv);
 }
 
 struct Conv3Args {
@@ -554,6 +588,35 @@
         hipLaunchKernelGGL((split_gemm_add_kernel<SP, BM, BN, PREFETCH, true>), grid, dim3(THREADS), 0, s, x, x2, w.p[0], w.p[1], w.p[2], w.scale, bias, y, M, K, N);
     else
         hipLaunchKernelGGL((split_gemm_add_kernel<SP, BM, BN, PREFETCH, false>), grid, dim3(THREADS), 0, s, x, x2, w.p[0], w.p[1], w.p[2], w.scale, bias, y, M, K, N);
+    return hipGetLastError() == hipSuccess ? TF_MSDA_OK : TF_MSDA_ERR_LAUNCH;
+}
+
+std::atomic<int> g_add2_prefetch{-1};
+int add2_prefetch()
+{
+    int v = g_add2_prefetch.load(std::memory_order_relaxed);
+    if (v < 0) {
+        const char *e = getenv("TF_LINEAR_ADD2_PREFETCH");
+        v = (e && e[0] == '1') ? 1 : 0;
+        g_add2_prefetch.store(v);
+    }
+    return v;
+}
+
+template <int SP, int BM, int BN>
+int launch_add2(const float *x, const float *x2, const Add2Out &v, const Add2Out &q, int M, int K, hipStream_t s)
+{
+    const int ntv = (v.n + BN - 1) / BN, ntiles = ntv + (q.n + BN - 1) / BN;
+    const long long groups = ((long long)M + 8 * BM - 1) / (8 * BM);
+    if (groups * 8 * ntiles > 0x7fffffffLL) return TF_MSDA_ERR_BAD_DIMS;
+    const dim3 grid((unsigned)(groups * 8 * ntiles));
+    const bool buf = fits_bufstore(M, v.n) && fits_bufstore(M, q.n);
+    auto go = [&](auto pf, auto bs) {
+        hipLaunchKernelGGL((split_gemm_add2_kernel<SP, BM, BN, decltype(pf)::value, decltype(bs)::value>), grid, dim3(THREADS), 0, s, x, x2, v, q,
+                           M, K, ntv, ntiles);
+    };
+    if (add2_prefetch()) buf ? go(std::true_type{}, std::true_type{}) : go(std::true_type{}, std::false_type{});
+    else buf ? go(std::false_type{}, std::true_type{}) : go(std::false_type{}, std::false_type{});
     return hipGetLastError() == hipSuccess ? TF_MSDA_OK : TF_MSDA_ERR_LAUNCH;
 }
 
@@ -712,6 +775,27 @@
     });
 }
 
+extern "C" int tf_linear_split_add2_f32(const float *x, const float *x2, const void *wv_hi, const void *wv_mid, const void *wv_lo,
+                                        const float *wv_scale, const float *bias_v, float *value, int Nv, const void *wq_hi,
+                                        const void *wq_mid, const void *wq_lo, const float *wq_scale, const float *bias_q, float *qproj,
+                                        int Nq, int64_t M, int K, void *stream)
+{
+    if (!x || !x2 || !value || !qproj) return TF_MSDA_ERR_NULL_POINTER;
+    Weight wv, wq;
+    const int sp = weight_scheme(wv_hi, wv_mid, wv_lo, wv_scale, wv), spq = weight_scheme(wq_hi, wq_mid, wq_lo, wq_scale, wq);
+    if (sp == 0 || spq == 0) return TF_MSDA_ERR_NULL_POINTER;
+    if (sp < 0 || spq != sp || M <= 0 || K <= 0 || Nv <= 0 || Nq <= 0 || (K % BK) != 0 || M > 0x7fffffffLL ||
+        ((reinterpret_cast<uintptr_t>(x) | reinterpret_cast<uintptr_t>(x2)) & 15))
+        return TF_MSDA_ERR_BAD_DIMS;
+    const Add2Out v{{wv.p[0], wv.p[1], wv.p[2]}, wv.scale, bias_v, value, Nv}, q{{wq.p[0], wq.p[1], wq.p[2]}, wq.scale, bias_q, qproj, Nq};
+    hipStream_t s = static_cast<hipStream_t>(stream);
+    return with_scheme(sp, [&](auto spc) {
+        constexpr int SP = decltype(spc)::value;
+        if (M <= 4096) return launch_add2<SP, 64, 64>(x, x2, v, q, (int)M, K, s);
+        return launch_add2<SP, 64, 128>(x, x2, v, q, (int)M, K, s);
+    });
+}
+
 extern "C" int tf_conv3x3_splitk_f32(const float *x, const void *w_hi, const void *w_mid, const void *w_lo, const float *w_scale,
                                      const float *bias, float *y, float *workspace, int ksplit, int nimg, int hin, int win, int cin,
                                      int cout, int stride, int relu, void *stream)
diff --git a/trackformer_amd/deformable_transformer.py b/trackformer_amd/deformable_transformer.py
--- a/trackformer_amd/deformable_transformer.py
+++ b/trackformer_amd/deformable_transformer.py
@@ -333,9 +333,18 @@
         inf = _inference(self)
         q, q_pos = (src, pos) if (inf and pos is not None and fused.pos_add_fused_enabled()) else (self.with_pos_embed(src, pos), None)
         if inf and fused.linear_ln_fused_enabled():
+            tail, done = None, []
+            if fused.enc_tail_fused_enabled() and fused.ffn_fused_enabled() and self.activation is F.relu:
+                layer_in = src
+
+                def tail(attn_out):
+                    y = fused.attn_ffn(attn_out, self.self_attn.output_proj, layer_in, self.norm1, self.linear1, self.linear2, self.norm2)
+                    if y is not None:
+                        done.append(True)
+                    return y
             src = self.self_attn(q, reference_points, src, spatial_shapes, padding_mask,
-                                 residual_norm=(src, self.norm1), query_pos=q_pos)
-            return self.forward_ffn(src)
+                                 residual_norm=(src, self.norm1), query_pos=q_pos, tail=tail)
+            return src if done else self.forward_ffn(src)
         src2 = self.self_attn(q, reference_points, src, spatial_shapes, padding_mask, query_pos=q_pos)
         src = fused.residual_norm(src, self.dropout1(src2), self.norm1, _inference(self))
         return self.forward_ffn(src)
diff --git a/trackformer_amd/fused.py b/trackformer_amd/fused.py
--- a/trackformer_amd/fused.py
+++ b/trackformer_amd/fused.py
@@ -377,6 +377,67 @@
     return y.view(x.shape)
 
 
+_enc_tail_fused = os.environ.get("TF_ENC_TAIL_FUSED", "0") not in ("", "0")
+
+
+def enc_tail_fused_enabled():
+    return _enc_tail_fused
+
+
+def set_enc_tail_fused(on):
+    global _enc_tail_fused, _route_epoch
+    prev, _enc_tail_fused = _enc_tail_fused, bool(on)
+    if prev != _enc_tail_fused:
+        _route_epoch += 1
+    return prev
+
+
+def attn_ffn(attn, out_proj, residual, norm1, linear1, linear2, norm2):
+    if not (_enc_tail_fused and _linln_fused and _ffn_fused and _split_linear and attn.is_cuda and attn.dtype == torch.float32):
+        return None
+    if _range_audit is not None:
+        return None
+    wo, w1, w2 = out_proj.weight, linear1.weight, linear2.weight
+    F_, D = w1.shape
+    if (D not in (256, 288) or attn.shape[-1] != D or tuple(wo.shape) != (D, D) or tuple(w2.shape) != (D, F_) or F_ % 16 or F_ < 128
+            or attn.numel() == 0):
+        return None
+    if not all(w.dtype == torch.float32 and w.is_contiguous() and w.device == attn.device for w in (wo, w1, w2)):
+        return None
+    if _routed(wo) != (_routed(w1) or _routed(w2)):
+        return None
+    if not all(n.elementwise_affine and tuple(n.normalized_shape) == (D,) for n in (norm1, norm2)):
+        return None
+    a = attn.reshape(-1, D)
+    if not a.is_contiguous():
+        a = a.contiguous()
+    M = a.shape[0]
+    if M < max(_FFN_FUSED_MIN_ROWS, _LINLN_MIN_ROWS) or (M + 128) * D * 4 > 0xFFFFFFFF:
+        return None
+    vecs = (out_proj.bias, linear1.bias, linear2.bias, norm1.weight, norm1.bias, norm2.weight, norm2.bias)
+    if not all(v is None or _param_ok(v, attn) for v in vecs):
+        return None
+    if residual.dtype != torch.float32 or residual.device != attn.device or residual.numel() != a.numel():
+        return None
+    residual = residual.reshape(-1, D)
+    if not residual.is_contiguous():
+        residual = residual.contiguous()
+    if (a.data_ptr() | residual.data_ptr()) & 15:
+        return None
+    po, p1, p2 = _packed_weight(wo, None), _packed_weight(w1, None), _packed_weight(w2, None)
+    if po is None or p1 is None or p2 is None:
+        return None
+    with torch.cuda.device(attn.device):
+        y = torch.empty((M, D), dtype=torch.float32, device=attn.device)
+        rc = _cabi.lib().tf_attn_ffn_fused_f32(a.data_ptr(), po.data_ptr(), _ptr(out_proj.bias), residual.data_ptr(),
+                                               norm1.weight.data_ptr(), norm1.bias.data_ptr(), float(norm1.eps), p1.data_ptr(),
+                                               _ptr(linear1.bias), p2.data_ptr(), _ptr(linear2.bias), norm2.weight.data_ptr(),
+                                               norm2.bias.data_ptr(), float(norm2.eps), y.data_ptr(), M, D, F_, _terms(),
+                                               _stream(attn.device))
+    _cabi.check(rc, "tf_attn_ffn_fused_f32")
+    return y.view(attn.shape)
+
+
 _stem_pool_fused = os.environ.get("TF_STEM_POOL_FUSED", "1") != "0"
 
 
@@ -526,6 +587,56 @@
                                                  _stream(x.device))
     _cabi.check(rc, "tf_linear_split_add_f32")
     return y.view(*x.shape[:-1], N)
+
+
+_enc_proj_merged = os.environ.get("TF_ENC_PROJ_MERGED", "1") != "0"
+_ENC_PROJ_MERGED_MIN_ROWS = int(os.environ.get("TF_ENC_PROJ_MERGED_MIN_ROWS", "4097"))
+
+
+def enc_proj_merged_enabled():
+    return _enc_proj_merged
+
+
+def set_enc_proj_merged(on):
+    global _enc_proj_merged, _route_epoch
+    prev, _enc_proj_merged = _enc_proj_merged, bool(on)
+    if prev != _enc_proj_merged:
+        _route_epoch += 1
+    return prev
+
+
+def linear_add2(x, x2, weight_v, bias_v, weight_q, bias_q):
+    if not (_enc_proj_merged and _pos_add_fused and _split_linear and x.is_cuda and x.dtype == torch.float32
+            and x2.dtype == torch.float32 and x2.shape == x.shape and x2.device == x.device):
+        return None
+    if not all(w.dtype == torch.float32 and w.dim() == 2 and w.is_contiguous() and w.device == x.device for w in (weight_v, weight_q)):
+        return None
+    if _routed(weight_v) != _routed(weight_q):
+        return None
+    (Nv, K), (Nq, Kq) = weight_v.shape, weight_q.shape
+    if Kq != K or x.shape[-1] != K or K % 32 or x.numel() == 0:
+        return None
+    for b, n in ((bias_v, Nv), (bias_q, Nq)):
+        if b is not None and not (b.dtype == torch.float32 and b.is_contiguous() and b.numel() == n and b.device == x.device):
+            return None
+    a, b = x.reshape(-1, K), x2.reshape(-1, K)
+    if a.shape[0] < _ENC_PROJ_MERGED_MIN_ROWS:
+        return None
+    a = a if a.is_contiguous() else a.contiguous()
+    b = b if b.is_contiguous() else b.contiguous()
+    pv, pq = _split_weight(weight_v), _split_weight(weight_q)
+    if (a.data_ptr() | b.data_ptr() | pv[0].data_ptr() | pv[1].data_ptr() | _ptr(pv[2]) | pq[0].data_ptr() | pq[1].data_ptr()
+            | _ptr(pq[2])) & 15:
+        return None
+    with torch.cuda.device(x.device):
+        value = torch.empty((a.shape[0], Nv), dtype=torch.float32, device=x.device)
+        qproj = torch.empty((a.shape[0], Nq), dtype=torch.float32, device=x.device)
+        rc = _cabi.lib().tf_linear_split_add2_f32(a.data_ptr(), b.data_ptr(), pv[0].data_ptr(), pv[1].data_ptr(), _ptr(pv[2]),
+                                                  _ptr(pv[3]), _ptr(bias_v), value.data_ptr(), Nv, pq[0].data_ptr(),
+                                                  pq[1].data_ptr(), _ptr(pq[2]), _ptr(pq[3]), _ptr(bias_q), qproj.data_ptr(), Nq,
+                                                  a.shape[0], K, _stream(x.device))
+    _cabi.check(rc, "tf_linear_split_add2_f32")
+    return value.view(*x.shape[:-1], Nv), qproj.view(*x.shape[:-1], Nq)
 
 
 def conv3x3(x, w_taps, bias, relu, stride):
@@ -1021,6 +1132,10 @@
 
 linear = _ranged("linear", lambda x, weight, *a, **k: (weight,), lambda x, *a, **k: (x,))(linear)
 linear_add = _ranged("linear_add", lambda x, x2, weight, *a, **k: (weight,), lambda x, x2, *a, **k: (x + x2,))(linear_add)
+linear_add2 = _ranged("linear_add2", lambda x, x2, weight_v, bias_v, weight_q, *a, **k: (weight_v, weight_q),
+                      lambda x, x2, *a, **k: (x, x + x2))(linear_add2)
+attn_ffn = _ranged("attn_ffn", lambda attn, out_proj, residual, norm1, linear1, linear2, *a, **k: (out_proj.weight, linear1.weight, linear2.weight),
+                   lambda attn, *a, **k: (attn,))(attn_ffn)
 ffn = _ranged("ffn", lambda x, linear1, linear2, *a, **k: (linear1.weight, linear2.weight), _ffn_acts)(ffn)
 linear_residual_norm = _ranged("linear_residual_norm", lambda x, linear, *a, **k: (linear.weight,), lambda x, *a, **k: (x,))(linear_residual_norm)
 stem_conv = _ranged("stem_conv", lambda x, weight, *a, **k: (weight,), lambda x, *a, **k: (x,))(stem_conv)
diff --git a/trackformer_amd/msda.py b/trackformer_amd/msda.py
--- a/trackformer_amd/msda.py
+++ b/trackformer_amd/msda.py
@@ -286,10 +286,10 @@
         constant_(self.output_proj.bias.data, 0.)
 
     def forward(self, query, reference_points, input_flatten, input_spatial_shapes,
-                input_padding_mask=None, query_attn_mask=None, residual_norm=None, query_pos=None):
+                input_padding_mask=None, query_attn_mask=None, residual_norm=None, query_pos=None, tail=None):
         if residual_norm is not None:
             out = self._forward(query, reference_points, input_flatten, input_spatial_shapes, input_padding_mask,
-                                query_attn_mask, residual_norm, query_pos)
+                                query_attn_mask, residual_norm, query_pos, tail)
             if isinstance(out, _Normed):
                 return out.value
             return fused.residual_norm(residual_norm[0], out, residual_norm[1], True)
@@ -297,7 +297,7 @@
                              None, query_pos)
 
     def _forward(self, query, reference_points, input_flatten, input_spatial_shapes, input_padding_mask, query_attn_mask,
-                 residual_norm, query_pos=None):
+                 residual_norm, query_pos=None, tail=None):
         N, Len_q, _ = query.shape
         N, Len_in, _ = input_flatten.shape
         hs = _host_shapes_of(input_spatial_shapes)
@@ -309,9 +309,18 @@
 
         M, L, P = self.n_heads, self.n_levels, self.n_points
         inference = not self.training and not torch.is_grad_enabled()
-        value = fused.module_linear(self.value_proj, input_flatten, inference)
-        if input_padding_mask is not None:
-            value = value.masked_fill(input_padding_mask[..., None], float(0))
+        value = qproj = None
+        if (FUSED_INFERENCE and inference and query_pos is not None and input_padding_mask is None and hs is not None
+                and query_attn_mask is None and fused.enc_proj_merged_enabled() and query.data_ptr() == input_flatten.data_ptr()
+                and query.shape == input_flatten.shape and query.stride() == input_flatten.stride()):
+            w, b = self._cat_proj.get(self)
+            both = fused.linear_add2(query, query_pos, self.value_proj.weight, self.value_proj.bias, w, b)
+            if both is not None:
+                value, qproj = both
+        if value is None:
+            value = fused.module_linear(self.value_proj, input_flatten, inference)
+            if input_padding_mask is not None:
+                value = value.masked_fill(input_padding_mask[..., None], float(0))
         value = value.view(N, Len_in, M, self.d_model // M)
 
         if (FUSED_INFERENCE and hs is not None and query_attn_mask is None and value.is_cuda
@@ -319,8 +328,7 @@
                 and not torch.is_grad_enabled() and reference_points.shape[-1] in (2, 4)
                 and (self.d_model // M) % 4 == 0 and P in (1, 2, 4, 8)):
             w, b = self._cat_proj.get(self)
-            qproj = None
-            if query_pos is not None:
+            if qproj is None and query_pos is not None:
                 qproj = fused.linear_add(query, query_pos, w, b)
                 if qproj is None:
                     query = query + query_pos
@@ -331,6 +339,10 @@
             output = ms_deform_attn_forward_fused(value, input_spatial_shapes, reference_points,
                                                   qproj, M, L, P)
             if residual_norm is not None:
+                if tail is not None:
+                    y = tail(output)
+                    if y is not None:
+                        return _Normed(y)
                 y = fused.linear_residual_norm(output, self.output_proj, residual_norm[0], residual_norm[1])
                 if y is not None:
                     return _Normed(y)
```
